# freudh/lbt

Measured on AMD Instinct MI355X. Metric: train-step samples/sec, ResNet-20 CIFAR-10 8-bit DFP, 1/2/4/8 MI355X, higher is better.
Workload: dtype int8; 1 GPU; ResNet-20 CIFAR-10 8-bit DFXP W/A/G train step (fwd+bwd+SGD-momentum+range update); global_batch=128, per_gpu_batch=128, parallelism=dp1, hip_graph=True, executor=fused, grad_range=-6, loss_diverged=False

## Files before the change

lbt_amd/csrc/conv_fused.h:

```cpp
#pragma once
#include "chain_flags.h"
#include "conv_epilogue.h"
#include "lds_tr.h"
#include "pk2.h"

namespace {
using namespace lbt;

#ifdef LBT_P1STUDY
#define LBT_TSS(i) LBT_TS(i)
#define LBT_TSB(i) do { if ((i) == 1) LBT_TS(4); else if ((i) == 2) LBT_TS(5); } while (0)
#else
#define LBT_TSS(i) do { } while (0)
#define LBT_TSB(i) LBT_TS(i)
#endif
constexpr int kBNW = 8;
constexpr int kBThreads = kBNW * 64;
__host__ __device__ constexpr int tile_rows(int CS) { return CS == 1 ? 8 : 4; }
__host__ __device__ constexpr int halo_iters(int TH) { return ((TH + 2) * 128 + kBThreads - 1) / kBThreads; }
template <int CS_, int TH_>
struct FusedTile {
  static constexpr int CS = CS_, TH = TH_, C = CS * 16, C4 = C / 4, W = 512 / C, Wp = W + 2, NT = CS;
  static constexpr int kMaxKS = (9 * CS + 3) / 4;
  static constexpr int NQ = TH * 128, J = (NQ + kBThreads - 1) / kBThreads, NPR = 2 * TH;
  static constexpr int kBIt = halo_iters(TH);
  static_assert(TH % 4 == 0 || TH == 2, "whole groups of 4 rows, or 2-row tiles");
};

template <int C, int KS, bool W4>
struct WImg {
  static constexpr int kBpf = W4 ? 8 : 16;
  static constexpr int kColB = KS * kBpf;
  static constexpr int kStride = kColB + 16;
  static constexpr int kBytes = C * kStride;
  static constexpr int kChunks = C * kColB / 16;
  static constexpr int kIt = (kChunks + kBThreads - 1) / kBThreads;
  static_assert(kColB % 16 == 0, "16-byte chunks within a column");
  LBT_DEV static void load(const int8_t* src, v4i (&v)[kIt]) {
#pragma unroll
    for (int it = 0; it < kIt; ++it) {
      const int i = (int)threadIdx.x + it * kBThreads;
      v[it] = *reinterpret_cast<const v4i*>(src + (int64_t)(i < kChunks ? i : 0) * 16);
    }
  }
  LBT_DEV static void store(int8_t* lds, const v4i (&v)[kIt]) {
#pragma unroll
    for (int it = 0; it < kIt; ++it) {
      const int i = (int)threadIdx.x + it * kBThreads;
      if (i < kChunks) {
        const int g = i * 16, col = g / kColB;
        *reinterpret_cast<v4i*>(lds + col * kStride + (g - col * kColB)) = v[it];
      }
    }
  }
  LBT_DEV static v4i frag(const int8_t* lds, int col, int slice) {
    if constexpr (W4)
      return unpack_i4x16(*reinterpret_cast<const v2i*>(lds + col * kStride + slice * 8));
    else
      return *reinterpret_cast<const v4i*>(lds + col * kStride + slice * 16);
  }
};

template <int C, int TH>
LBT_DEV void halo_pad_fill(int8_t* img, int row0, int H, int word) {
  constexpr int C4 = C / 4, W = 512 / C, Wp = W + 2;
  constexpr int kSide = (TH + 2) * 2 * C4;
  static_assert(kSide <= kBThreads && W * C4 <= kBThreads, "one padding word per thread and kind");
  const int t = kBThreads - 1 - (int)threadIdx.x;
  if (t < kSide) {
    const int hy = t / (2 * C4), side = (t / C4) & 1, q = t % C4;
    *reinterpret_cast<int*>(img + (hy * Wp + side * (W + 1)) * C + q * 4) = word;
  }
  if (t < W * C4) {
    if (row0 == 0) *reinterpret_cast<int*>(img + C + t * 4) = word;
    if (row0 + TH >= H) *reinterpret_cast<int*>(img + ((TH + 1) * Wp + 1) * C + t * 4) = word;
  }
}

LBT_DEV int mask_count(bool p) { return __builtin_popcountll(__builtin_amdgcn_ballot_w64(p)); }
LBT_DEV float max_raw(float a, float b) {
  float r;
  asm("v_max_f32 %0, %1, %2" : "=v"(r) : "v"(a), "v"(b));
  return r;
}
LBT_DEV void ov_count2(pf2 xm, float T1, float T2, int& c) {
  const pf2 n = xm * pk(-0x1.fffffep-1f, -0x1.fffffep-1f);
  const float a0 = max_raw(xm.x, n.x), a1 = max_raw(xm.y, n.y);
  c += mask_count(a0 >= T1) + mask_count(a1 >= T1) + ((mask_count(a0 >= T2) + mask_count(a1 >= T2)) << 16);
  asm volatile("" : "+s"(c));
}
LBT_DEV void ov_count2_pos(pf2 xm, float T1, float T2, int& c) {
  c += mask_count(xm.x >= T1) + mask_count(xm.y >= T1) + ((mask_count(xm.x >= T2) + mask_count(xm.y >= T2)) << 16);
  asm volatile("" : "+s"(c));
}
LBT_DEV void ov_stage_w(int i, int nq, int c, int* sh) {
  counts_stage_w(i, nq, c & 0xffff, (int)((unsigned)c >> 16), sh);
}
LBT_DEV float ov_thr(bool cnt, float T) { return cnt ? T : __builtin_nanf(""); }
constexpr int kOvNan = 0x7fc00000;
LBT_DEV float ov_thr(int nanmask, float T) { return __int_as_float(__float_as_int(T) | nanmask); }

LBT_DEV pf2 qfloor2(const QState& s, pf2 xm, pf2 u) {
  const pf2 v = xm + u;
  return pk(floorf(clip_q(s, v.x)), floorf(clip_q(s, v.y)));
}
LBT_DEV int pack4f(pf2 a, pf2 b) {
  const int c[4] = {(int)a.x, (int)a.y, (int)b.x, (int)b.y};
  return pack4_i8(c);
}

inline bool noise_ok(const lbt_qdesc& q) { return q.bits > 0 && q.stochastic && q.noise; }

}
```

lbt_amd/csrc/conv_fused_bwd.hip:

```cpp
#include "conv_fused.h"
#include "conv_wgrad_body.h"

using namespace lbt;

LBT_TRACE_SETTER(conv_bwd)

namespace {

struct ConvBwdArgs {
  lbt_chain_bwd_b b;
  const int8_t* wd;
  int ks, nslices, w4;
  lbt_qdesc qw;
  int H, W;
  const float* add_src;
  lbt_chain_bwd_a a;
};

template <int C, int TH, int WB>
struct BwdShared {
  int8_t w[WB];
  int8_t gq[(TH + 2) * (512 / C + 2) * C];
  float tile[TH * (512 / C) * (C + 4)];
  float pb[2 * C];
  int part[kBNW][(2 * 4 + 2) * C];
  int cnt[kBNW * 2 * 5];
};

template <int CS, int CF, int NB, bool W4, int WCS, int TH = tile_rows(CS)>
__global__ __launch_bounds__(kBThreads, (CS == 4 && TH >= 4) ? 2 : 4) void conv_bwd_kernel(ConvBwdArgs p, WgradArgs wa, uint32_t nwg) {
  using T = FusedTile<CS, TH>;
  constexpr int C = T::C, C4 = T::C4, NT = T::NT, W = T::W, Wp = T::Wp, kMaxKS = T::kMaxKS;
  constexpr int kBIt = T::kBIt, NPR = T::NPR, NQ = T::NQ, J = T::J;
  constexpr int WC = WCS ? WCS : 1;
  using WI = WImg<C, 4 * kMaxKS, W4>;
  union Smem {
    BwdShared<C, TH, WI::kBytes> b;
    WgradShared<WC, kBNW> w;
  };
  __shared__ __attribute__((aligned(16))) Smem sm;
  if (WCS != 0 && blockIdx.x < nwg) {
    conv_wgrad_body<WC, kBNW>(wa, blockIdx.x, sm.w);
    return;
  }
  BwdShared<C, TH, WI::kBytes>& sh = sm.b;
  LBT_TS(0);
  const lbt_chain_bwd_b& B = p.b;
  const lbt_chain_bwd_a& A = p.a;
  const int H = p.H;
  const uint32_t bid = blockIdx.x - nwg;
  const int tpi = H / TH;
  const int n = (int)(bid / (uint32_t)tpi), row0 = (int)(bid - (uint32_t)n * tpi) * TH;
  const int tid = threadIdx.x, lane = tid & 63, wave = tid >> 6;
  const int r = lane & 15, kg = lane >> 4;
  const int cq = (tid % C4) * 4;
  const int64_t img = (int64_t)n * H * W * C;

  static_assert(LBT_NSHARD == 32 && kBThreads == 512 && C % 16 == 0 && C / 16 <= kBNW, "statistics layout");
  constexpr int kSW = C / 16;
  long long sv[8][2];
  if (wave < kSW) {
    const int64_t* ps = B.sums + (int64_t)(8 * (lane >> 4)) * 4 * C + wave * 16 + (lane & 15);
#pragma unroll
    for (int i = 0; i < 8; ++i) {
      sv[i][0] = ps[(int64_t)i * 4 * C + 2 * C];
      sv[i][1] = ps[(int64_t)i * 4 * C + 3 * C];
    }
  }
  LBT_TSS(1);
  const int ylo = row0 > 0 ? row0 - 1 : 0, yhi = row0 + TH < H ? row0 + TH : H - 1;
  const int ngrp = (yhi - ylo + 1) * W * C4;
  int Gv[kBIt], Qv[kBIt];
  float4 Uv[kBIt];
#pragma unroll
  for (int it = 0; it < kBIt; ++it) {
    const int g = tid + it * kBThreads;
    const uint32_t off = g < ngrp ? (uint32_t)((ylo * W + g / C4) * C + cq) : 0u;
    Gv[it] = ld_i8x4(B.G, img + off);
    Qv[it] = ld_i8x4(B.qn_codes, img + off);
    Uv[it] = ld_f32x4(B.qo.noise, off);
  }
  v4i wimg[WI::kIt];
  WI::load(p.wd, wimg);
  float mu[4], sg[4], gam[2][4], bet[4];
#pragma unroll
  for (int k = 0; k < 4; ++k) {
    mu[k] = B.ms[cq + k];
    sg[k] = B.ms[C + cq + k];
#pragma unroll
    for (int b = 0; b < NB; ++b) gam[b][k] = (b == 0 ? A.b1 : A.b2).gb[cq + k];
    bet[k] = A.b1.gb[C + cq + k];
  }
  const QState sgq = qstate(B.qng), sn = qstate(B.qn), so = qstate(B.qo);
  QState qrg[2], qng[2];
#pragma unroll
  for (int b = 0; b < NB; ++b) {
    qrg[b] = qstate((b == 0 ? A.b1 : A.b2).qrg);
    qng[b] = qstate((b == 0 ? A.b1 : A.b2).qng);
  }
  const float r_inv = (CF & kAMaskR) ? qstate(A.b1.qr).inv_m : 0.f;
  const float scale = ldexpf(1.0f, -(frac_exp(B.qo) + frac_exp(p.qw)));
  LBT_TSS(2);

  if (wave < kSW) {
    long long SGi = 0, SGQi = 0;
#pragma unroll
    for (int i = 0; i < 8; ++i) {
      SGi += sv[i][0];
      SGQi += sv[i][1];
    }
    SGi = rows_total64(SGi);
    SGQi = rows_total64(SGQi);
    const int c = wave * 16 + (lane & 15);
    if (lane < 16) {
      const double s = (double)sn.inv_m, gsc = (double)sgq.inv_m, nn = (double)B.n;
      const double SG = (double)SGi, SGQ = (double)SGQi;
      const float m = B.ms[c], sig = B.ms[C + c];
      sh.pb[c] = (float)(gsc * SG / nn);
      sh.pb[C + c] = (float)(gsc * (s * SGQ - (double)m * SG) / (nn * (double)sig));
    }
  }
  LBT_TSS(3);
  __syncthreads();
  LBT_TSB(1);
  float rmg[4], rmgx[4];
  Recip rsg[4];
#pragma unroll
  for (int k = 0; k < 4; ++k) {
    rmg[k] = sh.pb[cq + k];
    rmgx[k] = sh.pb[C + cq + k];
    rsg[k] = recip(sg[k]);
  }
  pf2 mu2[2], sg2[2], rsc2[2], rmg2[2], rmgx2[2];
#pragma unroll
  for (int h = 0; h < 2; ++h) {
    mu2[h] = pk(mu[2 * h], mu[2 * h + 1]);
    sg2[h] = pk(rsg[2 * h].y, rsg[2 * h + 1].y);
    rsc2[h] = pk(rsg[2 * h].rc, rsg[2 * h + 1].rc);
    rmg2[h] = pk(rmg[2 * h], rmg[2 * h + 1]);
    rmgx2[h] = pk(rmgx[2 * h], rmgx[2 * h + 1]);
  }

  const int wu = __builtin_amdgcn_readfirstlane(wave);
  int ovq = 0;
  int s1[4] = {0, 0, 0, 0}, s2[4] = {0, 0, 0, 0};
#pragma unroll
  for (int it = 0; it < kBIt; ++it) {
    if (it * kBThreads + wu * 64 >= ngrp) break;
    const int g = tid + it * kBThreads;
    const int ry = g / (W * C4), x = g / C4 - ry * W;
    const int y = ylo + ry, hy = y - row0 + 1;
    const int pix = hy * Wp + x + 1;
    const bool own = hy >= 1 && hy <= TH;
    const int hyw = ylo + (it * kBThreads + wu * 64) / (W * C4) - row0 + 1;
    const int nanw = hyw >= 1 && hyw <= TH ? 0 : kOvNan;
    const float T1 = ov_thr(nanw, so.L), T2 = ov_thr(nanw, so.Lh);
    int G[4], q[4], c[4];
    unpack4_i8(Gv[it], G);
    unpack4_i8(Qv[it], q);
    const pf2 u[2] = {pk(Uv[it].x, Uv[it].y), pk(Uv[it].z, Uv[it].w)};
#pragma unroll
    for (int h = 0; h < 2; ++h) {
      const pf2 x1 = pcvt(q[2 * h], q[2 * h + 1]) * sn.inv_m;
      const pf2 x2 = x1 - mu2[h];
      const pf2 xh = pdiv_nz(x2, sg2[h], rsc2[h]);
      const pf2 gh = pcvt(G[2 * h], G[2 * h + 1]) * sgq.inv_m;
      const pf2 t1 = gh - rmg2[h];
      const pf2 t2 = xh * rmgx2[h];
      const pf2 dx = pdiv_nz(t1 - t2, sg2[h], rsc2[h]);
      const pf2 xm = dx * so.m;
      ov_count2(xm, T1, T2, ovq);
      const pf2 fl = qfloor2(so, xm, u[h]);
      c[2 * h] = (int)fl.x;
      c[2 * h + 1] = (int)fl.y;
    }
    *reinterpret_cast<int*>(sh.gq + pix * C + cq) = pack4_i8(c);
    if (own) {
      st_out(B.gq + img + (uint32_t)((y * W + x) * C + cq), pack4_i8(c));
#pragma unroll
      for (int k = 0; k < 4; ++k) {
        s1[k] += c[k];
        s2[k] += c[k] * c[k];
      }
    }
  }
  halo_pad_fill<C, TH>(sh.gq, row0, H, 0);
  WI::store(sh.w, wimg);
  __syncthreads();
  LBT_TSB(2);

  float4 av[J], ymv[J], urg[NB][J], ung[NB][J];
  int Rv[NB][J], qnv[NB][J];
#pragma unroll
  for (int j = 0; j < J; ++j) {
    const int q3 = tid + j * kBThreads;
    const int pix = (q3 < NQ ? q3 : 0) / C4;
    const uint32_t off = (uint32_t)(row0 * W * C + pix * C + cq);
    av[j] = p.add_src ? ld_f32x4(p.add_src, img + off) : make_float4(0.f, 0.f, 0.f, 0.f);
    if (CF & kAYMask) ymv[j] = ld_f32x4(A.y_mask, img + off);
#pragma unroll
    for (int b = 0; b < NB; ++b) {
      const lbt_bwd_branch& Bb = b == 0 ? A.b1 : A.b2;
      Rv[b][j] = ld_i8x4(Bb.R, img + off);
      qnv[b][j] = ld_i8x4(Bb.qn_codes, img + off);
      urg[b][j] = ld_f32x4(Bb.qrg.noise, off);
      ung[b][j] = ld_f32x4(Bb.qng.noise, off);
    }
  }

#pragma unroll
  for (int pi = 0; pi < (NPR + 7) / 8; ++pi) {
    const int pr = wave + 8 * pi;
    if (NPR % 8 && pr >= NPR) break;
    const int mt = pr / NT, nt = pr - mt * NT;
    const int m = mt * 16 + r;
    const int ly = m / W, px = m - ly * W;
    const int8_t* base = sh.gq + ((ly + 2) * Wp + px + 2) * C;
    v4i acc = v4i{0, 0, 0, 0};
    const int col = nt * 16 + r;
#pragma unroll
    for (int kk = 0; kk < kMaxKS; ++kk) {
      const int s = kk * 4 + kg;
      const int tap = s / CS, cs = s - tap * CS;
      const int kh = tap / 3, kw = tap - kh * 3;
      v4i a = *reinterpret_cast<const v4i*>(base - (kh * Wp + kw) * C + cs * 16);
      if (s >= 9 * CS) a = v4i{0, 0, 0, 0};
      acc = __builtin_amdgcn_mfma_i32_16x16x64_i8(a, WI::frag(sh.w, col, s), acc, 0, 0, 0);
    }
#pragma unroll
    for (int i = 0; i < 4; ++i) sh.tile[(mt * 16 + 4 * kg + i) * (C + 4) + nt * 16 + r] = (float)acc[i] * scale;
  }
  __syncthreads();
  LBT_TSB(3);

  int ov[2][2] = {{0, 0}, {0, 0}};
  int acc3[NB][4][4];
#pragma unroll
  for (int b = 0; b < NB; ++b)
#pragma unroll
    for (int s = 0; s < 4; ++s)
#pragma unroll
      for (int k = 0; k < 4; ++k) acc3[b][s][k] = 0;
  const bool has_add = p.add_src != nullptr;
  pf2 gam2a[NB][2], bet2a[2];
#pragma unroll
  for (int h = 0; h < 2; ++h) {
#pragma unroll
    for (int b = 0; b < NB; ++b) gam2a[b][h] = pk(gam[b][2 * h], gam[b][2 * h + 1]);
    bet2a[h] = pk(bet[2 * h], bet[2 * h + 1]);
  }
#pragma unroll
  for (int j = 0; j < J; ++j) {
    if (NQ % kBThreads && wu * 64 + j * kBThreads >= NQ) break;
    const int pix = (tid + j * kBThreads) / C4;
    const uint32_t off = (uint32_t)(row0 * W * C + pix * C + cq);
    const float4 t = *reinterpret_cast<const float4*>(sh.tile + pix * (C + 4) + cq);
    pf2 g[2] = {pk(t.x, t.y), pk(t.z, t.w)};
    if (has_add) {
      g[0] = g[0] + pk(av[j].x, av[j].y);
      g[1] = g[1] + pk(av[j].z, av[j].w);
    }
    int R1[4];
    unpack4_i8(Rv[0][j], R1);
    if (CF & kAYMask) {
      const float ym[4] = {ymv[j].x, ymv[j].y, ymv[j].z, ymv[j].w};
#pragma unroll
      for (int h = 0; h < 2; ++h)
        g[h] = pk(ym[2 * h] > 0.f ? g[h].x : 0.f, ym[2 * h + 1] > 0.f ? g[h].y : 0.f);
    } else if (CF & kAMaskR) {
#pragma unroll
      for (int h = 0; h < 2; ++h) {
        const pf2 xr = pcvt(R1[2 * h], R1[2 * h + 1]) * r_inv;
        const pf2 m1 = xr * gam2a[0][h];
        const pf2 yv = m1 + bet2a[h];
        g[h] = pk(yv.x > 0.f ? g[h].x : 0.f, yv.y > 0.f ? g[h].y : 0.f);
      }
    }
    if (CF & kAGmask) st_out4(A.gmask_out, (uint32_t)(img + off), make_float4(g[0].x, g[0].y, g[1].x, g[1].y));
#pragma unroll
    for (int b = 0; b < NB; ++b) {
      const lbt_bwd_branch& Bb = b == 0 ? A.b1 : A.b2;
      int R[4], qn[4], Gc[4];
      unpack4_i8(Rv[b][j], R);
      unpack4_i8(qnv[b][j], qn);
      const pf2 ur[2] = {pk(urg[b][j].x, urg[b][j].y), pk(urg[b][j].z, urg[b][j].w)};
      const pf2 un[2] = {pk(ung[b][j].x, ung[b][j].y), pk(ung[b][j].z, ung[b][j].w)};
#pragma unroll
      for (int h = 0; h < 2; ++h) {
        const pf2 xm = g[h] * qrg[b].m;
        ov_count2(xm, qrg[b].L, qrg[b].Lh, ov[b][0]);
        const pf2 f1 = qfloor2(qrg[b], xm, ur[h]);
        const pf2 gh = f1 * qrg[b].inv_m;
        const pf2 d = gh * gam2a[b][h];
        const pf2 dm = d * qng[b].m;
        ov_count2(dm, qng[b].L, qng[b].Lh, ov[b][1]);
        const pf2 f2c = qfloor2(qng[b], dm, un[h]);
        const int G2[2] = {(int)f1.x, (int)f1.y};
        Gc[2 * h] = (int)f2c.x;
        Gc[2 * h + 1] = (int)f2c.y;
#pragma unroll
        for (int i = 0; i < 2; ++i) {
          const int k = 2 * h + i;
          acc3[b][0][k] += G2[i] * R[k];
          acc3[b][1][k] += G2[i];
          acc3[b][2][k] += Gc[k];
          acc3[b][3][k] += Gc[k] * qn[k];
        }
      }
      st_out(Bb.gout + img + off, pack4_i8(Gc));
    }
  }

  {
    const bool own = (lane & 15) < C4;
    int* part = sh.part[wave] + cq + (lane >> 4);
#pragma unroll
    for (int b = 0; b < NB; ++b)
#pragma unroll
      for (int s = 0; s < 4; ++s) {
        const int t = chan_scatter4(acc3[b][s], C4);
        if (own) part[(b * 4 + s) * C] = t;
      }
    const int t1 = chan_scatter4(s1, C4), t2 = chan_scatter4(s2, C4);
    if (own) {
      part[8 * C] = t1;
      part[9 * C] = t2;
    }
  }
  ov_stage_w(0, 5, ovq, sh.cnt);
#pragma unroll
  for (int b = 0; b < NB; ++b) {
    ov_stage_w(1 + 2 * b, 5, ov[b][0], sh.cnt);
    ov_stage_w(2 + 2 * b, 5, ov[b][1], sh.cnt);
  }
  __syncthreads();
  LBT_TSB(4);
  counts_publish_nw<kBNW>(0, 5, B.qo, sh.cnt);
#pragma unroll
  for (int b = 0; b < NB; ++b) {
    const lbt_bwd_branch& Bb = b == 0 ? A.b1 : A.b2;
    counts_publish_nw<kBNW>(1 + 2 * b, 5, Bb.qrg, sh.cnt);
    counts_publish_nw<kBNW>(2 + 2 * b, 5, Bb.qng, sh.cnt);
  }
  const int shard = shard_id();
  for (int i = tid; i < (NB * 4 + 2) * C; i += kBThreads) {
    const int slot = i < NB * 4 * C ? i : 8 * C + (i - NB * 4 * C);
    long long v = 0;
#pragma unroll
    for (int w = 0; w < kBNW; ++w) v += sh.part[w][slot];
    if (!v) continue;
    int64_t* dst;
    if (i < NB * 4 * C) {
      const int b = i / (4 * C);
      dst = (b == 0 ? A.b1 : A.b2).sums + (int64_t)shard * 4 * C + (i - b * 4 * C);
    } else {
      if (!B.gcolsum) continue;
      dst = B.gcolsum + (int64_t)shard * 2 * C + (i - NB * 4 * C);
    }
    LBT_GADD((unsigned long long*)dst, (unsigned long long)v);
  }
  LBT_TSB(5);
}

}

extern "C" int lbt_conv_bwd_fused_i8(const lbt_conv_bwd* q, void* stream) {
  if (!q) return LBT_EINVAL;
  const lbt_conv_desc& d = q->d;
  const int C = d.Cin;
  if (!desc_ok(d) || d.KH != 3 || d.KW != 3 || d.SH != 1 || d.SW != 1 || d.PT != 1 || d.PB != 1 || d.PL != 1 ||
      d.PR != 1 || d.Ho != d.H || d.Wo != d.W || d.Cout != C || (C != 16 && C != 32 && C != 64) ||
      d.H % tile_rows(C / 16) || d.W * C != 512 || (int64_t)d.N * d.H * 512 >= ((int64_t)1 << 29))
    return LBT_EINVAL;
  const int CS = C / 16;
  const int64_t inner = (int64_t)d.H * d.W * C;
  const lbt_chain_bwd_b& b = q->b;
  if (!b.G || !b.qn_codes || !b.ms || !b.sums || !b.gq || b.dx || !noise_ok(b.qo) || b.C != C || b.rows != d.N ||
      b.inner != inner)
    return LBT_EINVAL;
  const lbt_chain_bwd_a& a = q->a;
  if (a.C != C || a.rows != d.N || a.inner != inner) return LBT_EINVAL;
  const int f = bwd_a_flags(a);
  if ((f & kAFused) != kAFused) return LBT_EINVAL;
  for (int br = 0; br < (a.has_b2 ? 2 : 1); ++br) {
    const lbt_bwd_branch& Bb = br ? a.b2 : a.b1;
    if (!noise_ok(Bb.qrg) || !noise_ok(Bb.qng) || !Bb.gb) return LBT_EINVAL;
  }
  if (q->ksd != 4 * ((9 * CS + 3) / 4) || !q->wd) return LBT_EINVAL;
  if (q->w4 && q->qw.bits > 4) return LBT_EINVAL;
  if (q->b.qo.bits > 8) return LBT_EINVAL;
  WgradArgs wa{};
  uint32_t wblocks = 0;
  int wcs = 0;
  if (q->w.slab) {
    const int e = wgrad_setup(q->w.xq, q->w.x_u8off, q->w.gq, q->w.d, q->w.slab, q->w.nsplit, q->w.nshard, wa, wblocks);
    if (e) return e;
    wcs = q->w.d.Cin / 16;
  }
  ConvBwdArgs p;
  p.b = b; p.wd = q->wd; p.ks = q->ksd; p.nslices = 9 * CS; p.w4 = q->w4; p.qw = q->qw;
  p.H = d.H; p.W = d.W; p.add_src = q->add_src; p.a = a;
  const int th = lbt_conv_fused_tile_rows(C, d.N, d.H);
  const int64_t tiles = (int64_t)d.N * (d.H / th);
  if (tiles + wblocks > 0x7fffffff) return LBT_EINVAL;
  const dim3 grid((unsigned)(tiles + wblocks));
  hipStream_t st = (hipStream_t)stream;
  const int nb = a.has_b2 ? 2 : 1;
#define LBT_BW_TH(CS_, CF_, NB_, WCS_, TH_)                                                                 \
  if (q->w4)                                                                                                \
    hipLaunchKernelGGL((conv_bwd_kernel<CS_, CF_, NB_, true, WCS_, TH_>), grid, dim3(kBThreads), 0, st, p, wa, wblocks); \
  else                                                                                                      \
    hipLaunchKernelGGL((conv_bwd_kernel<CS_, CF_, NB_, false, WCS_, TH_>), grid, dim3(kBThreads), 0, st, p, wa, wblocks);
#define LBT_BW(CS_, CF_, NB_, WCS_)                                                                  \
  if (CS == CS_ && f == (CF_) && nb == NB_ && wcs == WCS_) {                                       \
    if (CS_ == 1 && th == 4) {                                                                     \
      LBT_BW_TH(CS_, CF_, NB_, WCS_, (CS_ == 1 ? 4 : tile_rows(CS_)))                              \
    } else if (th == 2) {                                                                          \
      LBT_BW_TH(CS_, CF_, NB_, WCS_, 2)                                                            \
    } else {                                                                                       \
      LBT_BW_TH(CS_, CF_, NB_, WCS_, tile_rows(CS_))                                               \
    }                                                                                              \
    return (int)hipGetLastError();                                                                 \
  }
#define LBT_BW_CS(CS_)                                          \
  LBT_BW(CS_, kAFused | kAMaskR, 1, 0)                          \
  LBT_BW(CS_, kAFused | kAMaskR, 1, CS_)                        \
  LBT_BW(CS_, kAFused | kAYMask | kAGmask, 1, 0)                \
  LBT_BW(CS_, kAFused | kAYMask | kAGmask, 1, CS_)              \
  LBT_BW(CS_, kAFused | kAYMask, 2, 0)                          \
  LBT_BW(CS_, kAFused | kAYMask, 2, CS_)
  LBT_BW_CS(1)
  LBT_BW_CS(2)
  LBT_BW_CS(4)
  LBT_BW(1, kAFused | kAYMask, 1, 0)
  LBT_BW(1, kAFused | kAYMask, 1, 1)
  LBT_BW(1, kAFused | kAMaskR, 1, 2)
  LBT_BW(2, kAFused | kAMaskR, 1, 4)
#undef LBT_BW_CS
#undef LBT_BW
#undef LBT_BW_TH
  return LBT_EINVAL;
}

namespace {

struct ConvBwd2Args {
  lbt_chain_bwd_b b1, bs;
  const int8_t* wd1;
  const int8_t* wds;
  lbt_qdesc qw1, qws;
  int H;
  lbt_chain_bwd_a a;
};

template <int C, int TH>
struct Bwd2Shared {
  int8_t g1[(TH / 2 + 1) * 512];
  int8_t gs[(TH / 2) * 512];
  float tile[TH * (512 / C) * (C + 4)];
  float cst[2][5][2 * C];
  int part[kBNW][(2 * 4 + 8) * C];
  int cnt[kBNW * 2 * 6];
};

template <int CS, int CF, int NB, bool W4>
__global__ __launch_bounds__(kBThreads, CS == 1 ? 4 : 2) void conv_bwd2_kernel(ConvBwd2Args p) {
  constexpr int TH = tile_rows(CS);
  using T = FusedTile<CS, TH>;
  constexpr int C = T::C, C4 = T::C4, W = T::W, NT = T::NT, Cq = 2 * C, Cq4 = Cq / 4, CSq = 2 * CS;
  constexpr int Wq = W / 2, J = T::J;
  constexpr int kK1 = (9 * CSq + 3) / 4;
  constexpr int NG1 = (TH / 2 + 1) * Wq * Cq4, NGS = (TH / 2) * Wq * Cq4;
  constexpr int kIt = (NG1 + NGS + kBThreads - 1) / kBThreads;
  static_assert(NG1 % 64 == 0 && CSq <= 4 && LBT_NSHARD == 32 && 2 * Cq / 16 <= kBNW, "layout");
  __shared__ __attribute__((aligned(16))) Bwd2Shared<C, TH> sh;
  LBT_TS(0);
  const lbt_chain_bwd_a& A = p.a;
  const int H = p.H, Hq = H / 2;
  const uint32_t bid = blockIdx.x;
  const int tpi = H / TH;
  const int n = (int)(bid / (uint32_t)tpi), r0 = (int)(bid - (uint32_t)n * tpi) * TH, q0 = r0 / 2;
  const int tid = threadIdx.x, lane = tid & 63, wave = tid >> 6;
  const int r = lane & 15, kg = lane >> 4;
  const int cq = (tid % C4) * 4;
  const int cqq = (tid % Cq4) * 4;
  const int64_t img = (int64_t)n * H * W * C, imgq = (int64_t)n * Hq * Wq * Cq;

  constexpr int kSW = 2 * CSq;
  long long sv[8][2];
  if (wave < kSW) {
    const lbt_chain_bwd_b& Bb = wave < CSq ? p.b1 : p.bs;
    const int c = (wave % CSq) * 16 + (lane & 15);
    const int64_t* ps = Bb.sums + (int64_t)(8 * (lane >> 4)) * 4 * Cq + c;
#pragma unroll
    for (int i = 0; i < 8; ++i) {
      sv[i][0] = ps[(int64_t)i * 4 * Cq + 2 * Cq];
      sv[i][1] = ps[(int64_t)i * 4 * Cq + 3 * Cq];
    }
  }
  int Gv[kIt], Qv[kIt];
  float4 Uv[kIt];
#pragma unroll
  for (int it = 0; it < kIt; ++it) {
    const int g = tid + it * kBThreads;
    const bool r1 = g < NG1;
    const int gg = r1 ? g : g - NG1;
    const int pix = gg / Cq4, hy = pix / Wq, x = pix - hy * Wq;
    const int y = r1 ? q0 - 1 + hy : q0 + hy;
    const bool in = (r1 || gg < NGS) && (unsigned)y < (unsigned)Hq;
    const uint32_t off = in ? (uint32_t)((y * Wq + x) * Cq + cqq) : 0u;
    const lbt_chain_bwd_b& Bb = r1 ? p.b1 : p.bs;
    Gv[it] = ld_i8x4(Bb.G, imgq + off);
    Qv[it] = ld_i8x4(Bb.qn_codes, imgq + off);
    Uv[it] = ld_f32x4(Bb.qo.noise, off);
  }
  v4i bf1[kK1], bfs;
  {
    const int col = (wave % NT) * 16 + r;
#pragma unroll
    for (int kk = 0; kk < kK1; ++kk) {
      if constexpr (W4)
        bf1[kk] = unpack_i4x16(*reinterpret_cast<const v2i*>(p.wd1 + ((int64_t)col * (4 * kK1) + kk * 4 + kg) * 8));
      else
        bf1[kk] = *reinterpret_cast<const v4i*>(p.wd1 + ((int64_t)col * (4 * kK1) + kk * 4 + kg) * 16);
    }
    if constexpr (W4)
      bfs = unpack_i4x16(*reinterpret_cast<const v2i*>(p.wds + ((int64_t)col * 4 + kg) * 8));
    else
      bfs = *reinterpret_cast<const v4i*>(p.wds + ((int64_t)col * 4 + kg) * 16);
  }
  float gam[NB][4], bet[4];
#pragma unroll
  for (int k = 0; k < 4; ++k) {
#pragma unroll
    for (int b = 0; b < NB; ++b) gam[b][k] = (b == 0 ? A.b1 : A.b2).gb[cq + k];
    bet[k] = A.b1.gb[C + cq + k];
  }
  const QState so1 = qstate(p.b1.qo), sos = qstate(p.bs.qo);
  QState qrg[2], qng[2];
#pragma unroll
  for (int b = 0; b < NB; ++b) {
    qrg[b] = qstate((b == 0 ? A.b1 : A.b2).qrg);
    qng[b] = qstate((b == 0 ? A.b1 : A.b2).qng);
  }
  const float r_inv = (CF & kAMaskR) ? qstate(A.b1.qr).inv_m : 0.f;
  const float scale1 = ldexpf(1.0f, -(frac_exp(p.b1.qo) + frac_exp(p.qw1)));
  const float scale2 = ldexpf(1.0f, -(frac_exp(p.bs.qo) + frac_exp(p.qws)));

  if (wave < kSW) {
    long long SGi = 0, SGQi = 0;
#pragma unroll
    for (int i = 0; i < 8; ++i) {
      SGi += sv[i][0];
      SGQi += sv[i][1];
    }
    SGi = rows_total64(SGi);
    SGQi = rows_total64(SGQi);
    const int bn = wave < CSq ? 0 : 1, c = (wave % CSq) * 16 + (lane & 15);
    if (lane < 16) {
      const lbt_chain_bwd_b& Bb = bn == 0 ? p.b1 : p.bs;
      const double s = (double)qstate(Bb.qn).inv_m, gsc = (double)qstate(Bb.qng).inv_m, nn = (double)Bb.n;
      const double SG = (double)SGi, SGQ = (double)SGQi;
      const float m = Bb.ms[c], sig = Bb.ms[Cq + c];
      const Recip rc = recip(sig);
      sh.cst[bn][0][c] = m;
      sh.cst[bn][1][c] = sig;
      sh.cst[bn][2][c] = rc.rc;
      sh.cst[bn][3][c] = (float)(gsc * SG / nn);
      sh.cst[bn][4][c] = (float)(gsc * (s * SGQ - (double)m * SG) / (nn * (double)sig));
    }
  }
  const QState sn1 = qstate(p.b1.qn), sns = qstate(p.bs.qn), sg1 = qstate(p.b1.qng), sgs = qstate(p.bs.qng);
  __syncthreads();
  LBT_TS(1);

  int ova = 0, ovb = 0;
  const int g0w = __builtin_amdgcn_readfirstlane(tid) & ~63;
  int s1a[4] = {0, 0, 0, 0}, s2a[4] = {0, 0, 0, 0}, s1b[4] = {0, 0, 0, 0}, s2b[4] = {0, 0, 0, 0};
#pragma unroll
  for (int it = 0; it < kIt; ++it) {
    if (it * kBThreads >= NG1 + NGS) break;
    const int g = tid + it * kBThreads;
    const bool r1 = g < NG1;
    const int gg = r1 ? g : g - NG1;
    const bool valid = r1 || gg < NGS;
    const int pix = gg / Cq4, hy = pix / Wq, x = pix - hy * Wq;
    const int y = r1 ? q0 - 1 + hy : q0 + hy;
    const bool in = valid && (unsigned)y < (unsigned)Hq;
    const bool own = in && (!r1 || hy >= 1);
    const int bn = r1 ? 0 : 1;
    const QState& so = r1 ? so1 : sos;
    const QState& sn = r1 ? sn1 : sns;
    const QState& sgq = r1 ? sg1 : sgs;
    const float4 mu4 = *reinterpret_cast<const float4*>(&sh.cst[bn][0][cqq]);
    const float4 sg4 = *reinterpret_cast<const float4*>(&sh.cst[bn][1][cqq]);
    const float4 rc4 = *reinterpret_cast<const float4*>(&sh.cst[bn][2][cqq]);
    const float4 mg4 = *reinterpret_cast<const float4*>(&sh.cst[bn][3][cqq]);
    const float4 mx4 = *reinterpret_cast<const float4*>(&sh.cst[bn][4][cqq]);
    const pf2 mu2[2] = {pk(mu4.x, mu4.y), pk(mu4.z, mu4.w)}, sg2[2] = {pk(sg4.x, sg4.y), pk(sg4.z, sg4.w)};
    const pf2 rc2[2] = {pk(rc4.x, rc4.y), pk(rc4.z, rc4.w)}, mg2[2] = {pk(mg4.x, mg4.y), pk(mg4.z, mg4.w)};
    const pf2 mx2[2] = {pk(mx4.x, mx4.y), pk(mx4.z, mx4.w)};
    const float T1 = ov_thr(own, so.L), T2 = ov_thr(own, so.Lh);
    int G[4], q[4], c[4];
    unpack4_i8(Gv[it], G);
    unpack4_i8(Qv[it], q);
    const pf2 u[2] = {pk(Uv[it].x, Uv[it].y), pk(Uv[it].z, Uv[it].w)};
    int o = 0;
#pragma unroll
    for (int h = 0; h < 2; ++h) {
      const pf2 x1 = pcvt(q[2 * h], q[2 * h + 1]) * sn.inv_m;
      const pf2 x2 = x1 - mu2[h];
      const pf2 xh = pdiv_nz(x2, sg2[h], rc2[h]);
      const pf2 gh = pcvt(G[2 * h], G[2 * h + 1]) * sgq.inv_m;
      const pf2 t1 = gh - mg2[h];
      const pf2 t2 = xh * mx2[h];
      const pf2 dx = pdiv_nz(t1 - t2, sg2[h], rc2[h]);
      const pf2 xm = dx * so.m;
      ov_count2(xm, T1, T2, o);
      const pf2 fl = qfloor2(so, xm, u[h]);
      c[2 * h] = in ? (int)fl.x : 0;
      c[2 * h + 1] = in ? (int)fl.y : 0;
    }
    const int w = pack4_i8(c);
    const bool r1w = it * kBThreads + g0w < NG1;
    ova += r1w ? o : 0;
    ovb += r1w ? 0 : o;
    if (r1) {
      *reinterpret_cast<int*>(sh.g1 + pix * Cq + cqq) = w;
      if (own) {
        st_out(p.b1.gq + imgq + (uint32_t)((y * Wq + x) * Cq + cqq), w);
#pragma unroll
        for (int k = 0; k < 4; ++k) {
          s1a[k] += c[k];
          s2a[k] += c[k] * c[k];
        }
      }
    } else {
      if (valid) *reinterpret_cast<int*>(sh.gs + pix * Cq + cqq) = w;
      if (own) {
        st_out(p.bs.gq + imgq + (uint32_t)((y * Wq + x) * Cq + cqq), w);
#pragma unroll
        for (int k = 0; k < 4; ++k) {
          s1b[k] += c[k];
          s2b[k] += c[k] * c[k];
        }
      }
    }
  }
  __syncthreads();
  LBT_TS(2);

  float4 ymv[J], urg[NB][J], ung[NB][J];
  int Rv[NB][J], qnv[NB][J];
#pragma unroll
  for (int j = 0; j < J; ++j) {
    const int pix = (tid + j * kBThreads) / C4;
    const uint32_t off = (uint32_t)(r0 * W * C + pix * C + cq);
    if (CF & kAYMask) ymv[j] = ld_f32x4(A.y_mask, img + off);
#pragma unroll
    for (int b = 0; b < NB; ++b) {
      const lbt_bwd_branch& Bb = b == 0 ? A.b1 : A.b2;
      Rv[b][j] = ld_i8x4(Bb.R, img + off);
      qnv[b][j] = ld_i8x4(Bb.qn_codes, img + off);
      urg[b][j] = ld_f32x4(Bb.qrg.noise, off);
      ung[b][j] = ld_f32x4(Bb.qng.noise, off);
    }
  }

#pragma unroll
  for (int pi = 0; pi < TH / 4; ++pi) {
    const int pr = wave + 8 * pi;
    const int mt = pr / NT, nt = pr - mt * NT;
    const int m = mt * 16 + r;
    const int ly = m / W, px = m - ly * W;
    v4i acc = v4i{0, 0, 0, 0}, acc2 = v4i{0, 0, 0, 0};
#pragma unroll
    for (int kk = 0; kk < kK1; ++kk) {
      const int s = kk * 4 + kg;
      const int tap = s / CSq, cs = s - tap * CSq;
      const int kh = tap / 3, kw = tap - kh * 3;
      const bool ok = s < 9 * CSq && ((ly - kh) & 1) == 0 && ((px - kw) & 1) == 0 && px >= kw;
      const int lr = ((ly - kh) >> 1) + 1, ox = (px - kw) >> 1;
      v4i a = *reinterpret_cast<const v4i*>(sh.g1 + (ok ? (lr * Wq + ox) * Cq + cs * 16 : 0));
      if (!ok) a = v4i{0, 0, 0, 0};
      acc = __builtin_amdgcn_mfma_i32_16x16x64_i8(a, bf1[kk], acc, 0, 0, 0);
    }
    {
      const bool ok = kg < CSq && (ly & 1) == 0 && (px & 1) == 0;
      v4i a = *reinterpret_cast<const v4i*>(sh.gs + (ok ? ((ly >> 1) * Wq + (px >> 1)) * Cq + kg * 16 : 0));
      if (!ok) a = v4i{0, 0, 0, 0};
      acc2 = __builtin_amdgcn_mfma_i32_16x16x64_i8(a, bfs, acc2, 0, 0, 0);
    }
#pragma unroll
    for (int i = 0; i < 4; ++i) {
      const float v = (float)acc[i] * scale1, add = (float)acc2[i] * scale2;
      sh.tile[(mt * 16 + 4 * kg + i) * (C + 4) + nt * 16 + r] = v + add;
    }
  }
  __syncthreads();
  LBT_TS(3);

  int ov[2][2] = {{0, 0}, {0, 0}};
  int acc3[NB][4][4];
#pragma unroll
  for (int b = 0; b < NB; ++b)
#pragma unroll
    for (int s = 0; s < 4; ++s)
#pragma unroll
      for (int k = 0; k < 4; ++k) acc3[b][s][k] = 0;
  pf2 gam2a[NB][2], bet2a[2];
#pragma unroll
  for (int h = 0; h < 2; ++h) {
#pragma unroll
    for (int b = 0; b < NB; ++b) gam2a[b][h] = pk(gam[b][2 * h], gam[b][2 * h + 1]);
    bet2a[h] = pk(bet[2 * h], bet[2 * h + 1]);
  }
#pragma unroll
  for (int j = 0; j < J; ++j) {
    const int pix = (tid + j * kBThreads) / C4;
    const uint32_t off = (uint32_t)(r0 * W * C + pix * C + cq);
    const float4 t = *reinterpret_cast<const float4*>(sh.tile + pix * (C + 4) + cq);
    pf2 g[2] = {pk(t.x, t.y), pk(t.z, t.w)};
    int R1[4];
    unpack4_i8(Rv[0][j], R1);
    if (CF & kAYMask) {
      const float ym[4] = {ymv[j].x, ymv[j].y, ymv[j].z, ymv[j].w};
#pragma unroll
      for (int h = 0; h < 2; ++h)
        g[h] = pk(ym[2 * h] > 0.f ? g[h].x : 0.f, ym[2 * h + 1] > 0.f ? g[h].y : 0.f);
    } else if (CF & kAMaskR) {
#pragma unroll
      for (int h = 0; h < 2; ++h) {
        const pf2 xr = pcvt(R1[2 * h], R1[2 * h + 1]) * r_inv;
        const pf2 m1 = xr * gam2a[0][h];
        const pf2 yv = m1 + bet2a[h];
        g[h] = pk(yv.x > 0.f ? g[h].x : 0.f, yv.y > 0.f ? g[h].y : 0.f);
      }
    }
    if (CF & kAGmask) st_out4(A.gmask_out, (uint32_t)(img + off), make_float4(g[0].x, g[0].y, g[1].x, g[1].y));
#pragma unroll
    for (int b = 0; b < NB; ++b) {
      const lbt_bwd_branch& Bb = b == 0 ? A.b1 : A.b2;
      int R[4], qn[4], Gc[4];
      unpack4_i8(Rv[b][j], R);
      unpack4_i8(qnv[b][j], qn);
      const pf2 ur[2] = {pk(urg[b][j].x, urg[b][j].y), pk(urg[b][j].z, urg[b][j].w)};
      const pf2 un[2] = {pk(ung[b][j].x, ung[b][j].y), pk(ung[b][j].z, ung[b][j].w)};
#pragma unroll
      for (int h = 0; h < 2; ++h) {
        const pf2 xm = g[h] * qrg[b].m;
        ov_count2(xm, qrg[b].L, qrg[b].Lh, ov[b][0]);
        const pf2 f1 = qfloor2(qrg[b], xm, ur[h]);
        const pf2 gh = f1 * qrg[b].inv_m;
        const pf2 d = gh * gam2a[b][h];
        const pf2 dm = d * qng[b].m;
        ov_count2(dm, qng[b].L, qng[b].Lh, ov[b][1]);
        const pf2 f2c = qfloor2(qng[b], dm, un[h]);
        const int G2[2] = {(int)f1.x, (int)f1.y};
        Gc[2 * h] = (int)f2c.x;
        Gc[2 * h + 1] = (int)f2c.y;
#pragma unroll
        for (int i = 0; i < 2; ++i) {
          const int k = 2 * h + i;
          acc3[b][0][k] += G2[i] * R[k];
          acc3[b][1][k] += G2[i];
          acc3[b][2][k] += Gc[k];
          acc3[b][3][k] += Gc[k] * qn[k];
        }
      }
      st_out(Bb.gout + img + off, pack4_i8(Gc));
    }
  }

  {
    const bool own = (lane & 15) < C4;
    int* part = sh.part[wave] + cq + (lane >> 4);
#pragma unroll
    for (int b = 0; b < NB; ++b)
#pragma unroll
      for (int s = 0; s < 4; ++s) {
        const int t = chan_scatter4(acc3[b][s], C4);
        if (own) part[(b * 4 + s) * C] = t;
      }
    const bool ownq = (lane & 15) < Cq4;
    int* pq = sh.part[wave] + NB * 4 * C + cqq + (lane >> 4);
    const int t1 = chan_scatter4(s1a, Cq4), t2 = chan_scatter4(s2a, Cq4);
    const int t3 = chan_scatter4(s1b, Cq4), t4 = chan_scatter4(s2b, Cq4);
    if (ownq) {
      pq[0] = t1;
      pq[Cq] = t2;
      pq[2 * Cq] = t3;
      pq[3 * Cq] = t4;
    }
  }
  constexpr int NQ = 2 + 2 * NB;
  ov_stage_w(0, NQ, ova, sh.cnt);
  ov_stage_w(1, NQ, ovb, sh.cnt);
#pragma unroll
  for (int b = 0; b < NB; ++b) {
    ov_stage_w(2 + 2 * b, NQ, ov[b][0], sh.cnt);
    ov_stage_w(3 + 2 * b, NQ, ov[b][1], sh.cnt);
  }
  __syncthreads();
  LBT_TS(4);
  counts_publish_nw<kBNW>(0, NQ, p.b1.qo, sh.cnt);
  counts_publish_nw<kBNW>(1, NQ, p.bs.qo, sh.cnt);
#pragma unroll
  for (int b = 0; b < NB; ++b) {
    const lbt_bwd_branch& Bb = b == 0 ? A.b1 : A.b2;
    counts_publish_nw<kBNW>(2 + 2 * b, NQ, Bb.qrg, sh.cnt);
    counts_publish_nw<kBNW>(3 + 2 * b, NQ, Bb.qng, sh.cnt);
  }
  const int shard = shard_id();
  for (int i = tid; i < NB * 4 * C + 4 * Cq; i += kBThreads) {
    long long v = 0;
#pragma unroll
    for (int w = 0; w < kBNW; ++w) v += sh.part[w][i];
    if (!v) continue;
    int64_t* dst;
    if (i < NB * 4 * C) {
      const int b = i / (4 * C);
      dst = (b == 0 ? A.b1 : A.b2).sums + (int64_t)shard * 4 * C + (i - b * 4 * C);
    } else {
      const int k = i - NB * 4 * C;
      const lbt_chain_bwd_b& Bb = k < 2 * Cq ? p.b1 : p.bs;
      if (!Bb.gcolsum) continue;
      dst = Bb.gcolsum + (int64_t)shard * 2 * Cq + (k < 2 * Cq ? k : k - 2 * Cq);
    }
    LBT_GADD((unsigned long long*)dst, (unsigned long long)v);
  }
  LBT_TS(5);
}

}

extern "C" int lbt_conv_bwd2_fused_i8(const lbt_conv_bwd2* q, void* stream) {
  if (!q) return LBT_EINVAL;
  const lbt_conv_desc &d1 = q->d1, &ds = q->ds;
  const int C = d1.Cin, Cq = d1.Cout;
  if (!desc_ok(d1) || !desc_ok(ds) || d1.KH != 3 || d1.KW != 3 || d1.SH != 2 || d1.SW != 2 || d1.PT != 0 ||
      d1.PL != 0 || ds.KH != 1 || ds.KW != 1 || ds.SH != 2 || ds.SW != 2 || ds.PT != 0 || ds.PL != 0 ||
      (C != 16 && C != 32) || Cq != 2 * C || d1.W * C != 512 || d1.H % 2 || d1.W % 2 || d1.Ho * 2 != d1.H ||
      d1.Wo * 2 != d1.W || d1.H % tile_rows(C / 16) || ds.N != d1.N || ds.H != d1.H || ds.W != d1.W || ds.Cin != C ||
      ds.Cout != Cq || ds.Ho != d1.Ho || ds.Wo != d1.Wo || (int64_t)d1.N * d1.H * 512 >= ((int64_t)1 << 29))
    return LBT_EINVAL;
  const int CS = C / 16;
  const int64_t inq = (int64_t)d1.Ho * d1.Wo * Cq;
  const lbt_chain_bwd_b* bb[2] = {&q->b1, &q->bs};
  for (int i = 0; i < 2; ++i) {
    const lbt_chain_bwd_b& b = *bb[i];
    if (!b.G || !b.qn_codes || !b.ms || !b.sums || !b.gq || b.dx || !noise_ok(b.qo) || b.C != Cq || b.rows != d1.N ||
        b.inner != inq)
      return LBT_EINVAL;
  }
  const lbt_chain_bwd_a& a = q->a;
  if (a.C != C || a.rows != d1.N || a.inner != (int64_t)d1.H * d1.W * C) return LBT_EINVAL;
  const int f = bwd_a_flags(a);
  if ((f & kAFused) != kAFused) return LBT_EINVAL;
  for (int br = 0; br < (a.has_b2 ? 2 : 1); ++br) {
    const lbt_bwd_branch& Bb = br ? a.b2 : a.b1;
    if (!noise_ok(Bb.qrg) || !noise_ok(Bb.qng) || !Bb.gb) return LBT_EINVAL;
  }
  if (q->ksd1 != 4 * ((9 * 2 * CS + 3) / 4) || q->ksds != 4 || !q->wd1 || !q->wds) return LBT_EINVAL;
  if (q->w4 && (q->qw1.bits > 4 || q->qws.bits > 4)) return LBT_EINVAL;
  if (q->b1.qo.bits > 8 || q->bs.qo.bits > 8) return LBT_EINVAL;
  ConvBwd2Args p;
  p.b1 = q->b1; p.bs = q->bs; p.wd1 = q->wd1; p.wds = q->wds; p.qw1 = q->qw1; p.qws = q->qws; p.H = d1.H; p.a = a;
  const int64_t tiles = (int64_t)d1.N * (d1.H / tile_rows(CS));
  if (tiles > 0x7fffffff || (int64_t)d1.N * d1.H * d1.W * C >= ((int64_t)1 << 31)) return LBT_EINVAL;
  hipStream_t st = (hipStream_t)stream;
  const int nb = a.has_b2 ? 2 : 1;
#define LBT_B2(CS_, CF_, NB_)                                                                              \
  if (CS == CS_ && f == (CF_) && nb == NB_) {                                                              \
    if (q->w4)                                                                                             \
      hipLaunchKernelGGL((conv_bwd2_kernel<CS_, CF_, NB_, true>), dim3((unsigned)tiles), dim3(kBThreads), 0, st, p); \
    else                                                                                                   \
      hipLaunchKernelGGL((conv_bwd2_kernel<CS_, CF_, NB_, false>), dim3((unsigned)tiles), dim3(kBThreads), 0, st, p); \
    return (int)hipGetLastError();                                                                         \
  }
  LBT_B2(1, kAFused | kAYMask | kAGmask, 1)
  LBT_B2(2, kAFused | kAYMask | kAGmask, 1)
  LBT_B2(1, kAFused | kAYMask, 1)
  LBT_B2(2, kAFused | kAYMask, 1)
#undef LBT_B2
  return LBT_EINVAL;
}
```

lbt_amd/csrc/conv_fused_fwd.h:

```cpp
#pragma once
#include "conv_fused.h"

namespace lbt {
int conv_fwd_fused_infer(const lbt_conv_fwd* q, hipStream_t st);
int conv_fwd2_fused_infer(const lbt_conv_fwd2* q, hipStream_t st);
}

namespace {

struct ConvFwdArgs {
  lbt_chain_fwd c;
  const int8_t* wf;
  const int32_t* wcolsum;
  lbt_qdesc qw;
  int H;
  int8_t* yq;
  lbt_qdesc qout;
  int64_t* ychsum;
};

template <int C, int TH, int WB, bool INF = false>
struct FwdShared {
  int8_t w[WB];
  int8_t x[(TH + 2) * (512 / C + 2) * C];
  float tile[TH * (512 / C) * (C + 4)];
  float cst[2][2][C];
  int part[INF ? 1 : kBNW][2 * C];
  int cnt[INF ? 1 : kBNW * 2 * 4];
};

__host__ __device__ constexpr int fwd_waves(int CS, int NB, bool W4, int TH, bool INF) {
  return (CS == 4 && TH >= 4) ? 2 : (CS == 2 && NB == 2 && W4 && TH == 2 && !INF) ? 6 : 4;
}
template <int CS, int NB, int F, bool W4, int TH = tile_rows(CS), bool INF = false>
__global__ __launch_bounds__(kBThreads, fwd_waves(CS, NB, W4, TH, INF)) void conv_fwd_fused_kernel(ConvFwdArgs p) {
  using T = FusedTile<CS, TH>;
  constexpr int C = T::C, C4 = T::C4, NT = T::NT, W = T::W, Wp = T::Wp, kMaxKS = T::kMaxKS;
  constexpr int kBIt = T::kBIt, NQ = T::NQ, J = T::J, NPR = T::NPR;
  using WI = WImg<C, 4 * kMaxKS, W4>;
  __shared__ __attribute__((aligned(16))) FwdShared<C, TH, WI::kBytes, INF> sh;
  LBT_TS(0);
  const lbt_chain_fwd& a = p.c;
  const int H = p.H;
  const uint32_t bid = blockIdx.x;
  const int tpi = H / TH;
  const int n = (int)(bid / (uint32_t)tpi), row0 = (int)(bid - (uint32_t)n * tpi) * TH;
  const int tid = threadIdx.x, lane = tid & 63, wave = tid >> 6;
  const int r = lane & 15, kg = lane >> 4;
  const int cq = (tid % C4) * 4;
  const int64_t img = (int64_t)n * H * W * C;
  constexpr bool RES = (F & kFRes) != 0, YST = (F & kFY) != 0;

  static_assert(LBT_NSHARD == 32 && kBThreads == 512 && (NB * C) % 16 == 0 && NB * C / 16 <= kBNW,
                "moments layout");
  constexpr int kSW = NB * C / 16;
  long long sv[8][2];
  float rmean = 0.f, rvar = 0.f;
  if constexpr (INF) {
    if (tid < NB * C) {
      const lbt_bn_norm& nb = tid < C ? a.b1.nrm : a.b2.nrm;
      rmean = nb.run_mean[tid % C];
      rvar = nb.run_var[tid % C];
    }
  } else if (wave < kSW) {
    const int bc = wave * 16 + (lane & 15), b = bc / C, c = bc - b * C;
    const int64_t* cs = (b == 0 ? a.b1 : a.b2).nrm.chsum + (int64_t)(8 * (lane >> 4)) * 2 * C + c;
#pragma unroll
    for (int i = 0; i < 8; ++i) {
      sv[i][0] = cs[(int64_t)i * 2 * C];
      sv[i][1] = cs[(int64_t)i * 2 * C + C];
    }
  }
  const int ylo = row0 > 0 ? row0 - 1 : 0, yhi = row0 + TH < H ? row0 + TH : H - 1;
  const int ngrp = (yhi - ylo + 1) * W * C4;
  int qv[NB][kBIt];
  float4 rv[kBIt], nrv[NB][kBIt], nov[kBIt];
#pragma unroll
  for (int it = 0; it < kBIt; ++it) {
    const int g = tid + it * kBThreads;
    const uint32_t off = g < ngrp ? (uint32_t)((ylo * W + g / C4) * C + cq) : 0u;
#pragma unroll
    for (int b = 0; b < NB; ++b) {
      const lbt_chain_branch& Bb = b == 0 ? a.b1 : a.b2;
      qv[b][it] = ld_i8x4(Bb.nrm.q, img + off);
      nrv[b][it] = ld_f32x4(Bb.qr.noise, off);
    }
    if constexpr (RES) rv[it] = ld_f32x4(a.res, img + off);
    nov[it] = ld_f32x4(a.qo1.noise, off);
  }
  v4i wimg[WI::kIt];
  WI::load(p.wf, wimg);
  const int bcol = (wave % NT) * 16 + r;
  const int corr = 128 * p.wcolsum[bcol];
  float gam[NB][4], bet[NB][4];
#pragma unroll
  for (int b = 0; b < NB; ++b)
#pragma unroll
    for (int k = 0; k < 4; ++k) {
      gam[b][k] = (b == 0 ? a.b1 : a.b2).gb[cq + k];
      bet[b][k] = (b == 0 ? a.b1 : a.b2).gb[C + cq + k];
    }
  QState qr[2];
  float sn[2];
#pragma unroll
  for (int b = 0; b < NB; ++b) {
    qr[b] = qstate((b == 0 ? a.b1 : a.b2).qr);
    sn[b] = qscale((b == 0 ? a.b1 : a.b2).nrm.qn);
  }
  const QState so1 = qstate(a.qo1), sq = qstate(p.qout);
  const float scale = ldexpf(1.0f, -(frac_exp(a.qo1) + frac_exp(p.qw)));

  if constexpr (INF) {
    if (tid < NB * C) {
      const float eps = (tid < C ? a.b1.nrm : a.b2.nrm).eps;
      sh.cst[tid / C][0][tid % C] = rmean;
      sh.cst[tid / C][1][tid % C] = sqrtf(rvar + eps);
    }
  } else if (wave < kSW) {
    long long S1 = 0, S2 = 0;
#pragma unroll
    for (int i = 0; i < 8; ++i) {
      S1 += sv[i][0];
      S2 += sv[i][1];
    }
    S1 = rows_total64(S1);
    S2 = rows_total64(S2);
    const int bc = wave * 16 + (lane & 15), b = bc / C, c = bc - b * C;
    if (lane < 16) {
    const lbt_bn_norm& nb = b == 0 ? a.b1.nrm : a.b2.nrm;
    const double s = ldexp(1.0, -frac_exp(nb.qn));
    const double mean_d = (double)S1 * s / (double)nb.n;
    const double var_d = (double)S2 * (s * s) / (double)nb.n - mean_d * mean_d;
    const float m = (float)mean_d, vv = (float)var_d;
    const float sigma = sqrtf(vv + nb.eps);
    sh.cst[b][0][c] = m;
    sh.cst[b][1][c] = sigma;
    if (bid == 0) {
      if (nb.ms) { nb.ms[c] = m; nb.ms[C + c] = sigma; }
      if (nb.run_mean) {
        nb.run_mean[c] = nb.momentum * nb.run_mean[c] + nb.one_minus_momentum * m;
        nb.run_var[c] = nb.momentum * nb.run_var[c] + nb.one_minus_momentum * vv;
      }
    }
    }
  }
  __syncthreads();
  LBT_TS(1);
  float pm[NB][4];
  Recip ps[NB][4];
#pragma unroll
  for (int b = 0; b < NB; ++b)
#pragma unroll
    for (int k = 0; k < 4; ++k) {
      pm[b][k] = sh.cst[b][0][cq + k];
      ps[b][k] = recip(sh.cst[b][1][cq + k]);
    }
  pf2 pm2[NB][2], psy2[NB][2], psr2[NB][2], gam2[NB][2], bet2[NB][2];
#pragma unroll
  for (int b = 0; b < NB; ++b)
#pragma unroll
    for (int h = 0; h < 2; ++h) {
      pm2[b][h] = pk(pm[b][2 * h], pm[b][2 * h + 1]);
      psy2[b][h] = pk(ps[b][2 * h].y, ps[b][2 * h + 1].y);
      psr2[b][h] = pk(ps[b][2 * h].rc, ps[b][2 * h + 1].rc);
      gam2[b][h] = pk(gam[b][2 * h], gam[b][2 * h + 1]);
      bet2[b][h] = pk(bet[b][2 * h], bet[b][2 * h + 1]);
    }

  int wu = wave;
  if constexpr (!INF) wu = __builtin_amdgcn_readfirstlane(wave);
  int ovr[2] = {0, 0}, ovx = 0;
#pragma unroll
  for (int it = 0; it < kBIt; ++it) {
    if (it * kBThreads + wu * 64 >= ngrp) break;
    const int g = tid + it * kBThreads;
    const int ry = g / (W * C4), x = g / C4 - ry * W;
    const int y = ylo + ry, hy = y - row0 + 1;
    const int pix = hy * Wp + x + 1;
    const bool own = hy >= 1 && hy <= TH;
    const int hyw = ylo + (it * kBThreads + wu * 64) / (W * C4) - row0 + 1;
    const int nanw = hyw >= 1 && hyw <= TH ? 0 : kOvNan;
    const uint32_t e = (uint32_t)((y * W + x) * C + cq);
    pf2 v[2];
    float T1[2], T2[2];
    if constexpr (!INF) {
#pragma unroll
      for (int b = 0; b < NB; ++b) {
        T1[b] = ov_thr(nanw, qr[b].L);
        T2[b] = ov_thr(nanw, qr[b].Lh);
      }
    }
#pragma unroll
    for (int b = 0; b < NB; ++b) {
      const lbt_chain_branch& Bb = b == 0 ? a.b1 : a.b2;
      int q[4];
      unpack4_i8(qv[b][it], q);
      const pf2 u[2] = {pk(nrv[b][it].x, nrv[b][it].y), pk(nrv[b][it].z, nrv[b][it].w)};
      pf2 fl[2];
#pragma unroll
      for (int h = 0; h < 2; ++h) {
        const pf2 x1 = pcvt(q[2 * h], q[2 * h + 1]) * sn[b];
        const pf2 x2 = x1 - pm2[b][h];
        const pf2 t = pdiv_nz(x2, psy2[b][h], psr2[b][h]);
        const pf2 xm = t * qr[b].m;
        if constexpr (!INF) ov_count2(xm, T1[b], T2[b], ovr[b]);
        fl[h] = qfloor2(qr[b], xm, u[h]);
        const pf2 xr = fl[h] * qr[b].inv_m;
        const pf2 m1 = xr * gam2[b][h];
        const pf2 tt = m1 + bet2[b][h];
        v[h] = b ? v[h] + tt : tt;
      }
      if (own && (!INF || Bb.rout)) st_out(Bb.rout + img + e, pack4f(fl[0], fl[1]));
    }
    if constexpr (RES) {
      v[0] = v[0] + pk(rv[it].x, rv[it].y);
      v[1] = v[1] + pk(rv[it].z, rv[it].w);
    }
#pragma unroll
    for (int h = 0; h < 2; ++h) v[h] = pk(v[h].x > 0.f ? v[h].x : 0.f, v[h].y > 0.f ? v[h].y : 0.f);
    if (YST && own) st_out4(a.y, (uint32_t)(img + e), make_float4(v[0].x, v[0].y, v[1].x, v[1].y));
    const pf2 uo[2] = {pk(nov[it].x, nov[it].y), pk(nov[it].z, nov[it].w)};
    const float X1 = ov_thr(nanw, so1.L), X2 = ov_thr(nanw, so1.Lh);
    int co[4];
#pragma unroll
    for (int h = 0; h < 2; ++h) {
      const pf2 xm = v[h] * so1.m;
      if constexpr (!INF) ov_count2_pos(xm, X1, X2, ovx);
      const pf2 w = xm + uo[h];
      co[2 * h] = floor_i(fminf(w.x, so1.Lm1));
      co[2 * h + 1] = floor_i(fminf(w.y, so1.Lm1));
    }
    const int cw = pack4_i8(co) ^ (int)0x80808080;
    *reinterpret_cast<int*>(sh.x + pix * C + cq) = cw;
    if (own && (!INF || a.o1)) st_out((int8_t*)a.o1 + img + e, cw);
  }
  halo_pad_fill<C, TH>(sh.x, row0, H, (int)0x80808080);
  WI::store(sh.w, wimg);
  __syncthreads();
  LBT_TS(2);
  float4 u3[J];
#pragma unroll
  for (int j = 0; j < J; ++j) {
    const int q3 = tid + j * kBThreads;
    u3[j] = ld_f32x4(p.qout.noise, (uint32_t)(row0 * W * C + ((q3 < NQ ? q3 : 0) / C4) * C + cq));
  }

#pragma unroll
  for (int pi = 0; pi < (NPR + 7) / 8; ++pi) {
    const int pr = wave + 8 * pi;
    if (NPR % 8 && pr >= NPR) break;
    const int mt = pr / NT, nt = pr - mt * NT;
    const int m = mt * 16 + r;
    const int ly = m / W, px = m - ly * W;
    const int8_t* base = sh.x + (ly * Wp + px) * C;
    v4i acc = v4i{0, 0, 0, 0};
#pragma unroll
    for (int kk = 0; kk < kMaxKS; ++kk) {
      const int s = kk * 4 + kg;
      const int tap = s / CS, cs = s - tap * CS;
      const int kh = tap / 3, kw = tap - kh * 3;
      v4i av = *reinterpret_cast<const v4i*>(base + (kh * Wp + kw) * C + cs * 16);
      if (s >= 9 * CS) av = v4i{0, 0, 0, 0};
      acc = __builtin_amdgcn_mfma_i32_16x16x64_i8(av, WI::frag(sh.w, nt * 16 + r, s), acc, 0, 0, 0);
    }
#pragma unroll
    for (int i = 0; i < 4; ++i)
      sh.tile[(mt * 16 + 4 * kg + i) * (C + 4) + nt * 16 + r] = (float)(acc[i] + corr) * scale;
  }
  __syncthreads();
  LBT_TS(3);

  int ovq = 0;
  int s1[4] = {0, 0, 0, 0}, s2[4] = {0, 0, 0, 0};
#pragma unroll
  for (int j = 0; j < J; ++j) {
    if (NQ % kBThreads && (INF ? tid : wu * 64) + j * kBThreads >= NQ) break;
    const int pix3 = (tid + j * kBThreads) / C4;
    const float4 t = *reinterpret_cast<const float4*>(sh.tile + pix3 * (C + 4) + cq);
    const pf2 tv[2] = {pk(t.x, t.y), pk(t.z, t.w)};
    const pf2 u[2] = {pk(u3[j].x, u3[j].y), pk(u3[j].z, u3[j].w)};
    pf2 fl[2];
#pragma unroll
    for (int h = 0; h < 2; ++h) {
      const pf2 xm = tv[h] * sq.m;
      if constexpr (!INF) ov_count2(xm, sq.L, sq.Lh, ovq);
      fl[h] = qfloor2(sq, xm, u[h]);
    }
    const int c[4] = {(int)fl[0].x, (int)fl[0].y, (int)fl[1].x, (int)fl[1].y};
    if constexpr (!INF) {
#pragma unroll
      for (int k = 0; k < 4; ++k) {
        s1[k] += c[k];
        s2[k] += c[k] * c[k];
      }
    }
    st_out(p.yq + img + (uint32_t)(row0 * W * C + pix3 * C + cq), pack4_i8(c));
  }
  if constexpr (!INF) {
    {
      const int t1 = chan_scatter4(s1, C4), t2 = chan_scatter4(s2, C4);
      if ((lane & 15) < C4) {
        sh.part[wave][cq + (lane >> 4)] = t1;
        sh.part[wave][C + cq + (lane >> 4)] = t2;
      }
    }
#pragma unroll
    for (int b = 0; b < NB; ++b) ov_stage_w(b, 4, ovr[b], sh.cnt);
    ov_stage_w(2, 4, ovx, sh.cnt);
    ov_stage_w(3, 4, ovq, sh.cnt);
    __syncthreads();
    LBT_TS(4);
#pragma unroll
    for (int b = 0; b < NB; ++b) counts_publish_nw<kBNW>(b, 4, (b == 0 ? a.b1 : a.b2).qr, sh.cnt);
    counts_publish_nw<kBNW>(2, 4, a.qo1, sh.cnt);
    counts_publish_nw<kBNW>(3, 4, p.qout, sh.cnt);
    if (p.ychsum && tid < 2 * C) {
      long long t = 0;
#pragma unroll
      for (int w = 0; w < kBNW; ++w) t += sh.part[w][tid];
      if (t) LBT_GADD((unsigned long long*)&p.ychsum[(int64_t)shard_id() * 2 * C + tid], (unsigned long long)t);
    }
  }
  LBT_TS(5);
}

constexpr int kTH2 = 4;

struct ConvFwd2Args {
  lbt_chain_fwd c;
  const int8_t* wf1;
  const int8_t* wfs;
  const int32_t* wcolsum1;
  const int32_t* wcolsums;
  lbt_qdesc qw1, qws;
  int H;
  int8_t* yq1;
  int8_t* yqs;
  lbt_qdesc qout1, qouts;
  int64_t* ychsum1;
  int64_t* ychsums;
};

template <int C, bool INF = false>
struct Fwd2Shared {
  int8_t xa[(2 * kTH2 + 1) * 512];
  int8_t xs[kTH2 * 256];
  float tile[2][kTH2 * (256 / C) * (2 * C + 4)];
  float cst[2][C];
  int part[INF ? 1 : kBNW][2 * 2 * 2 * C];
  int cnt[INF ? 1 : kBNW * 2 * 5];
};

template <int CS, bool W4, bool INF = false>
__global__ __launch_bounds__(kBThreads, CS == 1 ? 4 : 2) void conv_fwd2_kernel(ConvFwd2Args p) {
  using T = FusedTile<CS, 2 * kTH2>;
  constexpr int C = T::C, C4 = T::C4, W = T::W, Cq = 2 * C, Cq4 = Cq / 4, Wq = W / 2, NTq = Cq / 16;
  constexpr int kK1 = T::kMaxKS;
  constexpr int NG = (2 * kTH2 + 1) * W * C4;
  constexpr int kIt = (NG + kBThreads - 1) / kBThreads;
  static_assert(kTH2 * Wq * Cq == 2 * 1024 && C / 16 <= kBNW, "layout");
  __shared__ __attribute__((aligned(16))) Fwd2Shared<C, INF> sh;
  LBT_TS(0);
  const lbt_chain_fwd& a = p.c;
  const int H = p.H, Hq = H / 2;
  const uint32_t bid = blockIdx.x;
  const int tpi = Hq / kTH2;
  const int n = (int)(bid / (uint32_t)tpi), oy0 = (int)(bid - (uint32_t)n * tpi) * kTH2, y0 = 2 * oy0;
  const int tid = threadIdx.x, lane = tid & 63, wave = tid >> 6;
  const int r = lane & 15, kg = lane >> 4;
  const int cq = (tid % C4) * 4, cqq = (tid % Cq4) * 4;
  const int64_t img = (int64_t)n * H * W * C, imgq = (int64_t)n * Hq * Wq * Cq;

  constexpr int kSW = C / 16;
  long long sv[8][2];
  float rmean = 0.f, rvar = 0.f;
  if constexpr (INF) {
    if (tid < C) {
      rmean = a.b1.nrm.run_mean[tid];
      rvar = a.b1.nrm.run_var[tid];
    }
  } else if (wave < kSW) {
    const int c = wave * 16 + (lane & 15);
    const int64_t* cs = a.b1.nrm.chsum + (int64_t)(8 * (lane >> 4)) * 2 * C + c;
#pragma unroll
    for (int i = 0; i < 8; ++i) {
      sv[i][0] = cs[(int64_t)i * 2 * C];
      sv[i][1] = cs[(int64_t)i * 2 * C + C];
    }
  }
  int qv[kIt];
  float4 rv[kIt], nrv[kIt], no1[kIt], no2[kIt];
#pragma unroll
  for (int it = 0; it < kIt; ++it) {
    const int g = tid + it * kBThreads;
    const int pix = g / C4, hy = pix / W, x = pix - hy * W;
    const int y = y0 + hy;
    const bool in = g < NG && y < H;
    const uint32_t off = in ? (uint32_t)((y * W + x) * C + cq) : 0u;
    qv[it] = ld_i8x4(a.b1.nrm.q, img + off);
    nrv[it] = ld_f32x4(a.b1.qr.noise, off);
    rv[it] = ld_f32x4(a.res, img + off);
    no1[it] = ld_f32x4(a.qo1.noise, off);
    no2[it] = ld_f32x4(a.qo2.noise, off);
  }
  const int mt = wave / NTq, nt = wave - mt * NTq;
  const int bcol = nt * 16 + r;
  v4i bf1[kK1], bfs;
#pragma unroll
  for (int kk = 0; kk < kK1; ++kk) {
    if constexpr (W4)
      bf1[kk] = unpack_i4x16(*reinterpret_cast<const v2i*>(p.wf1 + ((int64_t)bcol * (4 * kK1) + kk * 4 + kg) * 8));
    else
      bf1[kk] = *reinterpret_cast<const v4i*>(p.wf1 + ((int64_t)bcol * (4 * kK1) + kk * 4 + kg) * 16);
  }
  if constexpr (W4)
    bfs = unpack_i4x16(*reinterpret_cast<const v2i*>(p.wfs + ((int64_t)bcol * 4 + kg) * 8));
  else
    bfs = *reinterpret_cast<const v4i*>(p.wfs + ((int64_t)bcol * 4 + kg) * 16);
  const int corr1 = 128 * p.wcolsum1[bcol], corr2 = 128 * p.wcolsums[bcol];
  float gam[4], bet[4];
#pragma unroll
  for (int k = 0; k < 4; ++k) {
    gam[k] = a.b1.gb[cq + k];
    bet[k] = a.b1.gb[C + cq + k];
  }
  const QState qr = qstate(a.b1.qr), so1 = qstate(a.qo1), so2 = qstate(a.qo2);
  const QState sq1 = qstate(p.qout1), sqs = qstate(p.qouts);
  const float sn = qscale(a.b1.nrm.qn);
  const float scale1 = ldexpf(1.0f, -(frac_exp(a.qo1) + frac_exp(p.qw1)));
  const float scale2 = ldexpf(1.0f, -(frac_exp(a.qo2) + frac_exp(p.qws)));

  if constexpr (INF) {
    if (tid < C) {
      sh.cst[0][tid] = rmean;
      sh.cst[1][tid] = sqrtf(rvar + a.b1.nrm.eps);
    }
  } else if (wave < kSW) {
    long long S1 = 0, S2 = 0;
#pragma unroll
    for (int i = 0; i < 8; ++i) {
      S1 += sv[i][0];
      S2 += sv[i][1];
    }
    S1 = rows_total64(S1);
    S2 = rows_total64(S2);
    const int c = wave * 16 + (lane & 15);
    if (lane < 16) {
      const lbt_bn_norm& nb = a.b1.nrm;
      const double s = ldexp(1.0, -frac_exp(nb.qn));
      const double mean_d = (double)S1 * s / (double)nb.n;
      const double var_d = (double)S2 * (s * s) / (double)nb.n - mean_d * mean_d;
      const float m = (float)mean_d, vv = (float)var_d;
      const float sigma = sqrtf(vv + nb.eps);
      sh.cst[0][c] = m;
      sh.cst[1][c] = sigma;
      if (bid == 0) {
        if (nb.ms) { nb.ms[c] = m; nb.ms[C + c] = sigma; }
        if (nb.run_mean) {
          nb.run_mean[c] = nb.momentum * nb.run_mean[c] + nb.one_minus_momentum * m;
          nb.run_var[c] = nb.momentum * nb.run_var[c] + nb.one_minus_momentum * vv;
        }
      }
    }
  }
  __syncthreads();
  LBT_TS(1);
  pf2 pm2[2], psy2[2], psr2[2], gam2[2], bet2[2];
#pragma unroll
  for (int h = 0; h < 2; ++h) {
    const Recip r0 = recip(sh.cst[1][cq + 2 * h]), r1 = recip(sh.cst[1][cq + 2 * h + 1]);
    pm2[h] = pk(sh.cst[0][cq + 2 * h], sh.cst[0][cq + 2 * h + 1]);
    psy2[h] = pk(r0.y, r1.y);
    psr2[h] = pk(r0.rc, r1.rc);
    gam2[h] = pk(gam[2 * h], gam[2 * h + 1]);
    bet2[h] = pk(bet[2 * h], bet[2 * h + 1]);
  }

  int ovr = 0, ovx = 0, ovs = 0;
#pragma unroll
  for (int it = 0; it < kIt; ++it) {
    if (it * kBThreads >= NG) break;
    const int g = tid + it * kBThreads;
    const int pix = g / C4, hy = pix / W, x = pix - hy * W;
    const int y = y0 + hy;
    const bool valid = g < NG;
    const bool in = valid && y < H;
    const bool own = in && hy < 2 * kTH2;
    const uint32_t e = (uint32_t)((y * W + x) * C + cq);
    int q[4];
    unpack4_i8(qv[it], q);
    const pf2 u[2] = {pk(nrv[it].x, nrv[it].y), pk(nrv[it].z, nrv[it].w)};
    const float T1 = ov_thr(own, qr.L), T2 = ov_thr(own, qr.Lh);
    pf2 fl[2], v[2];
#pragma unroll
    for (int h = 0; h < 2; ++h) {
      const pf2 x1 = pcvt(q[2 * h], q[2 * h + 1]) * sn;
      const pf2 x2 = x1 - pm2[h];
      const pf2 t = pdiv_nz(x2, psy2[h], psr2[h]);
      const pf2 xm = t * qr.m;
      if constexpr (!INF) ov_count2(xm, T1, T2, ovr);
      fl[h] = qfloor2(qr, xm, u[h]);
      const pf2 xr = fl[h] * qr.inv_m;
      const pf2 m1 = xr * gam2[h];
      v[h] = m1 + bet2[h];
    }
    if (own && (!INF || a.b1.rout)) st_out(a.b1.rout + img + e, pack4f(fl[0], fl[1]));
    v[0] = v[0] + pk(rv[it].x, rv[it].y);
    v[1] = v[1] + pk(rv[it].z, rv[it].w);
#pragma unroll
    for (int h = 0; h < 2; ++h) v[h] = pk(v[h].x > 0.f ? v[h].x : 0.f, v[h].y > 0.f ? v[h].y : 0.f);
    if (own) st_out4(a.y, (uint32_t)(img + e), make_float4(v[0].x, v[0].y, v[1].x, v[1].y));
    const pf2 u1[2] = {pk(no1[it].x, no1[it].y), pk(no1[it].z, no1[it].w)};
    const pf2 u2[2] = {pk(no2[it].x, no2[it].y), pk(no2[it].z, no2[it].w)};
    const float X1 = ov_thr(own, so1.L), X2 = ov_thr(own, so1.Lh);
    const float Z1 = ov_thr(own, so2.L), Z2 = ov_thr(own, so2.Lh);
    int c1[4], c2[4];
#pragma unroll
    for (int h = 0; h < 2; ++h) {
      const pf2 xm = v[h] * so1.m;
      if constexpr (!INF) ov_count2_pos(xm, X1, X2, ovx);
      const pf2 w1 = xm + u1[h];
      c1[2 * h] = floor_i(fminf(w1.x, so1.Lm1));
      c1[2 * h + 1] = floor_i(fminf(w1.y, so1.Lm1));
      const pf2 zm = v[h] * so2.m;
      if constexpr (!INF) ov_count2_pos(zm, Z1, Z2, ovs);
      const pf2 w2 = zm + u2[h];
      c2[2 * h] = floor_i(fminf(w2.x, so2.Lm1));
      c2[2 * h + 1] = floor_i(fminf(w2.y, so2.Lm1));
    }
    const int cw1 = in ? (pack4_i8(c1) ^ (int)0x80808080) : (int)0x80808080;
    const int cw2 = in ? (pack4_i8(c2) ^ (int)0x80808080) : (int)0x80808080;
    if (valid) *reinterpret_cast<int*>(sh.xa + pix * C + cq) = cw1;
    if (own && !(hy & 1) && !(x & 1)) *reinterpret_cast<int*>(sh.xs + ((hy >> 1) * Wq + (x >> 1)) * C + cq) = cw2;
    if constexpr (INF) {
      if (own && a.o1) st_out((int8_t*)a.o1 + img + e, cw1);
      if (own && a.o2) st_out((int8_t*)a.o2 + img + e, cw2);
    } else if (own) {
      st_out((int8_t*)a.o1 + img + e, cw1);
      st_out((int8_t*)a.o2 + img + e, cw2);
    }
  }
  __syncthreads();
  LBT_TS(2);
  const uint32_t off3 = (uint32_t)(oy0 * Wq * Cq + (tid / Cq4) * Cq + cqq);
  const float4 un1 = ld_f32x4(p.qout1.noise, off3), uns = ld_f32x4(p.qouts.noise, off3);

  {
    const int m = mt * 16 + r;
    const int ly = m / Wq, px = m - ly * Wq;
    v4i acc = v4i{0, 0, 0, 0}, acc2 = v4i{0, 0, 0, 0};
#pragma unroll
    for (int kk = 0; kk < kK1; ++kk) {
      const int s = kk * 4 + kg;
      const int tap = s / CS, cs = s - tap * CS;
      const int kh = tap / 3, kw = tap - kh * 3;
      const int ix = 2 * px + kw;
      const bool okx = ix < W;
      v4i av = *reinterpret_cast<const v4i*>(sh.xa + (((2 * ly + kh) * W + (okx ? ix : 0)) * C + cs * 16));
      if (!okx) av = v4i{(int)0x80808080, (int)0x80808080, (int)0x80808080, (int)0x80808080};
      if (s >= 9 * CS) av = v4i{0, 0, 0, 0};
      acc = __builtin_amdgcn_mfma_i32_16x16x64_i8(av, bf1[kk], acc, 0, 0, 0);
    }
    {
      v4i av = *reinterpret_cast<const v4i*>(sh.xs + ((ly * Wq + px) * C + (kg < CS ? kg : 0) * 16));
      if (kg >= CS) av = v4i{0, 0, 0, 0};
      acc2 = __builtin_amdgcn_mfma_i32_16x16x64_i8(av, bfs, acc2, 0, 0, 0);
    }
#pragma unroll
    for (int i = 0; i < 4; ++i) {
      const int row = (mt * 16 + 4 * kg + i) * (Cq + 4) + nt * 16 + r;
      sh.tile[0][row] = (float)(acc[i] + corr1) * scale1;
      sh.tile[1][row] = (float)(acc2[i] + corr2) * scale2;
    }
  }
  __syncthreads();
  LBT_TS(3);

  int ovq[2] = {0, 0};
  int s1[2][4] = {{0, 0, 0, 0}, {0, 0, 0, 0}}, s2[2][4] = {{0, 0, 0, 0}, {0, 0, 0, 0}};
  {
    const int pix3 = tid / Cq4;
#pragma unroll
    for (int b = 0; b < 2; ++b) {
      const QState& sq = b ? sqs : sq1;
      const float4 un = b ? uns : un1;
      const float4 t = *reinterpret_cast<const float4*>(sh.tile[b] + pix3 * (Cq + 4) + cqq);
      const pf2 tv[2] = {pk(t.x, t.y), pk(t.z, t.w)};
      const pf2 u[2] = {pk(un.x, un.y), pk(un.z, un.w)};
      pf2 fl[2];
#pragma unroll
      for (int h = 0; h < 2; ++h) {
        const pf2 xm = tv[h] * sq.m;
        if constexpr (!INF) ov_count2(xm, sq.L, sq.Lh, ovq[b]);
        fl[h] = qfloor2(sq, xm, u[h]);
      }
      const int c[4] = {(int)fl[0].x, (int)fl[0].y, (int)fl[1].x, (int)fl[1].y};
      if constexpr (!INF) {
#pragma unroll
        for (int k = 0; k < 4; ++k) {
          s1[b][k] += c[k];
          s2[b][k] += c[k] * c[k];
        }
      }
      st_out((b ? p.yqs : p.yq1) + imgq + off3, pack4_i8(c));
    }
  }
  if constexpr (!INF) {
    {
      const bool ownq = (lane & 15) < Cq4;
#pragma unroll
      for (int b = 0; b < 2; ++b) {
        const int t1 = chan_scatter4(s1[b], Cq4), t2 = chan_scatter4(s2[b], Cq4);
        if (ownq) {
          sh.part[wave][b * 2 * Cq + cqq + (lane >> 4)] = t1;
          sh.part[wave][b * 2 * Cq + Cq + cqq + (lane >> 4)] = t2;
        }
      }
    }
    ov_stage_w(0, 5, ovr, sh.cnt);
    ov_stage_w(1, 5, ovx, sh.cnt);
    ov_stage_w(2, 5, ovs, sh.cnt);
    ov_stage_w(3, 5, ovq[0], sh.cnt);
    ov_stage_w(4, 5, ovq[1], sh.cnt);
    __syncthreads();
    LBT_TS(4);
    counts_publish_nw<kBNW>(0, 5, a.b1.qr, sh.cnt);
    counts_publish_nw<kBNW>(1, 5, a.qo1, sh.cnt);
    counts_publish_nw<kBNW>(2, 5, a.qo2, sh.cnt);
    counts_publish_nw<kBNW>(3, 5, p.qout1, sh.cnt);
    counts_publish_nw<kBNW>(4, 5, p.qouts, sh.cnt);
    if (tid < 4 * Cq) {
      long long t = 0;
#pragma unroll
      for (int w = 0; w < kBNW; ++w) t += sh.part[w][tid];
      int64_t* dst = tid < 2 * Cq ? p.ychsum1 : p.ychsums;
      if (t && dst) LBT_GADD((unsigned long long*)&dst[(int64_t)shard_id() * 2 * Cq + (tid % (2 * Cq))], (unsigned long long)t);
    }
  }
  LBT_TS(5);
}

}
```

lbt_amd/csrc/conv_fused_fwd.hip:

```cpp
#include "conv_fused_fwd.h"
#include "env.h"

using namespace lbt;

LBT_TRACE_SETTER(conv_fwd)

extern "C" int lbt_conv_fused_tile_rows(int32_t Cin, int64_t N, int32_t H) {
  if (Cin != 16 && Cin != 32 && Cin != 64) return -LBT_EINVAL;
  const int CS = Cin / 16;
  if (CS != 1) {
    static const int force23 = getenv_int("LBT_TILE_ROWS23", 0);
    if (force23 == 4 || H % 4) return 4;
    return (force23 == 2 || N * H / 4 < 256) ? 2 : 4;
  }
  static const int force = getenv_int("LBT_TILE_ROWS1", 0);
  if (force == 2 || force == 4 || force == 8) return H % force ? 8 : force;
  if (N * H / 8 >= 256 || H % 4) return 8;
  return (N * H / 4 < 256 && H % 2 == 0) ? 2 : 4;
}

static int frozen_chain(const lbt_chain_fwd& a) {
  const bool f1 = a.b1.nrm.frozen != 0, f2 = a.has_b2 ? a.b2.nrm.frozen != 0 : f1;
  return f1 != f2 ? -1 : (f1 ? 1 : 0);
}

extern "C" int lbt_conv_fwd_fused_i8(const lbt_conv_fwd* q, void* stream) {
  if (!q) return LBT_EINVAL;
  if (const int fz = frozen_chain(q->c)) return fz < 0 ? LBT_EINVAL : conv_fwd_fused_infer(q, (hipStream_t)stream);
  const lbt_conv_desc& d = q->d;
  const int C = d.Cin;
  if (!desc_ok(d) || d.KH != 3 || d.KW != 3 || d.SH != 1 || d.SW != 1 || d.PT != 1 || d.PB != 1 || d.PL != 1 ||
      d.PR != 1 || d.Ho != d.H || d.Wo != d.W || d.Cout != C || (C != 16 && C != 32 && C != 64) ||
      d.H % tile_rows(C / 16) || d.W * C != 512 || (int64_t)d.N * d.H * 512 >= ((int64_t)1 << 29))
    return LBT_EINVAL;
  const int CS = C / 16;
  const lbt_chain_fwd& a = q->c;
  const int64_t inner = (int64_t)d.H * d.W * C;
  if (a.C != C || a.rows != d.N || a.inner != inner || a.o2 || !a.o1 || a.o1_kind != LBT_OUT_U8OFF) return LBT_EINVAL;
  const int f = fwd_flags(a);
  constexpr int kNeed = kFQ | kFRout | kFRelu | kFO1 | kFStoch | kFU8;
  if ((f & kRt) || (f & kNeed) != kNeed || (f & (kFO2 | kFNoR))) return LBT_EINVAL;
  if (!noise_ok(a.qo1)) return LBT_EINVAL;
  for (int br = 0; br < (a.has_b2 ? 2 : 1); ++br) {
    const lbt_chain_branch& Bb = br ? a.b2 : a.b1;
    if (!noise_ok(Bb.qr) || !Bb.gb || !Bb.nrm.chsum || Bb.nrm.frozen) return LBT_EINVAL;
  }
  if (!q->yq || !noise_ok(q->qout) || !q->wcolsum || !q->wf) return LBT_EINVAL;
  if (q->ksf != 4 * ((9 * CS + 3) / 4)) return LBT_EINVAL;
  if (q->w4 && q->qw.bits > 4) return LBT_EINVAL;
  if (q->qout.bits > 8) return LBT_EINVAL;
  ConvFwdArgs p;
  p.c = a; p.wf = q->wf; p.wcolsum = q->wcolsum; p.qw = q->qw; p.H = d.H;
  p.yq = q->yq; p.qout = q->qout; p.ychsum = q->ychsum;
  const int th = lbt_conv_fused_tile_rows(C, d.N, d.H);
  const int64_t tiles = (int64_t)d.N * (d.H / th);
  if (tiles > 0x7fffffff) return LBT_EINVAL;
  const dim3 grid((unsigned)tiles);
  hipStream_t st = (hipStream_t)stream;
  const int nb = a.has_b2 ? 2 : 1;
  const int fl = f & ~kFU8 & ~kFStoch;
#define LBT_FW_TH(CS_, NB_, FL_, TH_)                                                                        \
  if (q->w4)                                                                                                 \
    hipLaunchKernelGGL((conv_fwd_fused_kernel<CS_, NB_, FL_, true, TH_>), grid, dim3(kBThreads), 0, st, p);    \
  else                                                                                                       \
    hipLaunchKernelGGL((conv_fwd_fused_kernel<CS_, NB_, FL_, false, TH_>), grid, dim3(kBThreads), 0, st, p);
#define LBT_FW(CS_, NB_, FL_)                                                                            \
  if (CS == CS_ && nb == NB_ && fl == ((FL_) & ~kFU8 & ~kFStoch)) {                                      \
    if (CS_ == 1 && th == 4) {                                                                           \
      LBT_FW_TH(CS_, NB_, FL_, (CS_ == 1 ? 4 : tile_rows(CS_)))                                          \
    } else if (th == 2) {                                                                                \
      LBT_FW_TH(CS_, NB_, FL_, 2)                                                                        \
    } else {                                                                                             \
      LBT_FW_TH(CS_, NB_, FL_, tile_rows(CS_))                                                           \
    }                                                                                                    \
    return (int)hipGetLastError();                                                                       \
  }
#define LBT_FW_CS(CS_)                                  \
  LBT_FW(CS_, 1, kNeed)                                 \
  LBT_FW(CS_, 1, kNeed | kFRes | kFY)                   \
  LBT_FW(CS_, 2, kNeed | kFY)
  LBT_FW(1, 1, kNeed)
  LBT_FW(1, 1, kNeed | kFRes | kFY)
  LBT_FW(1, 1, kNeed | kFY)
  LBT_FW_CS(2)
  LBT_FW_CS(4)
#undef LBT_FW_CS
#undef LBT_FW
#undef LBT_FW_TH
  return LBT_EINVAL;
}

extern "C" int lbt_conv_fwd2_fused_i8(const lbt_conv_fwd2* q, void* stream) {
  if (!q) return LBT_EINVAL;
  if (const int fz = frozen_chain(q->c)) return fz < 0 ? LBT_EINVAL : conv_fwd2_fused_infer(q, (hipStream_t)stream);
  const lbt_conv_desc &d1 = q->d1, &ds = q->ds;
  const int C = d1.Cin, Cq = d1.Cout;
  if (!desc_ok(d1) || !desc_ok(ds) || d1.KH != 3 || d1.KW != 3 || d1.SH != 2 || d1.SW != 2 || d1.PT != 0 ||
      d1.PL != 0 || ds.KH != 1 || ds.KW != 1 || ds.SH != 2 || ds.SW != 2 || ds.PT != 0 || ds.PL != 0 ||
      (C != 16 && C != 32) || Cq != 2 * C || d1.W * C != 512 || d1.H % 2 || d1.W % 2 || d1.Ho * 2 != d1.H ||
      d1.Wo * 2 != d1.W || d1.Ho % kTH2 || ds.N != d1.N || ds.H != d1.H || ds.W != d1.W || ds.Cin != C ||
      ds.Cout != Cq || ds.Ho != d1.Ho || ds.Wo != d1.Wo || (int64_t)d1.N * d1.H * 512 >= ((int64_t)1 << 29))
    return LBT_EINVAL;
  const int CS = C / 16;
  const lbt_chain_fwd& a = q->c;
  if (a.C != C || a.rows != d1.N || a.inner != (int64_t)d1.H * d1.W * C || a.has_b2 || !a.o1 || !a.o2 ||
      a.o1_kind != LBT_OUT_U8OFF || a.o2_kind != LBT_OUT_U8OFF || !a.res || !a.y)
    return LBT_EINVAL;
  const int f = fwd_flags(a);
  constexpr int kNeed = kFQ | kFRout | kFRelu | kFO1 | kFO2 | kFStoch | kFU8 | kFRes | kFY;
  if (f != kNeed) return LBT_EINVAL;
  if (!noise_ok(a.qo1) || !noise_ok(a.qo2) || !noise_ok(a.b1.qr) || !a.b1.gb || !a.b1.nrm.chsum || a.b1.nrm.frozen)
    return LBT_EINVAL;
  if (!q->yq1 || !q->yqs || !noise_ok(q->qout1) || !noise_ok(q->qouts) || !q->wcolsum1 || !q->wcolsums || !q->wf1 ||
      !q->wfs)
    return LBT_EINVAL;
  if (q->ksf1 != 4 * ((9 * CS + 3) / 4) || q->ksfs != 4) return LBT_EINVAL;
  if (q->w4 && (q->qw1.bits > 4 || q->qws.bits > 4)) return LBT_EINVAL;
  if (q->qout1.bits > 8 || q->qouts.bits > 8) return LBT_EINVAL;
  ConvFwd2Args p;
  p.c = a; p.wf1 = q->wf1; p.wfs = q->wfs; p.wcolsum1 = q->wcolsum1; p.wcolsums = q->wcolsums;
  p.qw1 = q->qw1; p.qws = q->qws; p.H = d1.H; p.yq1 = q->yq1; p.yqs = q->yqs; p.qout1 = q->qout1;
  p.qouts = q->qouts; p.ychsum1 = q->ychsum1; p.ychsums = q->ychsums;
  const int64_t tiles = (int64_t)d1.N * (d1.Ho / kTH2);
  if (tiles > 0x7fffffff || (int64_t)d1.N * d1.H * d1.W * C >= ((int64_t)1 << 31)) return LBT_EINVAL;
  hipStream_t st = (hipStream_t)stream;
#define LBT_F2(CS_)                                                                                           \
  if (CS == CS_) {                                                                                            \
    if (q->w4)                                                                                                \
      hipLaunchKernelGGL((conv_fwd2_kernel<CS_, true>), dim3((unsigned)tiles), dim3(kBThreads), 0, st, p);    \
    else                                                                                                      \
      hipLaunchKernelGGL((conv_fwd2_kernel<CS_, false>), dim3((unsigned)tiles), dim3(kBThreads), 0, st, p);   \
    return (int)hipGetLastError();                                                                            \
  }
  LBT_F2(1)
  LBT_F2(2)
#undef LBT_F2
  return LBT_EINVAL;
}
```

lbt_amd/csrc/conv_fused_infer.hip:

```cpp
#include "conv_fused_fwd.h"

using namespace lbt;

LBT_TRACE_SETTER(conv_infer)

namespace {

bool branch_ok(const lbt_chain_branch& b) {
  return b.nrm.frozen && b.nrm.q && b.nrm.run_mean && b.nrm.run_var && b.gb && noise_ok(b.qr) && !b.qr.counts;
}
bool qout_ok(const lbt_qdesc& q) { return noise_ok(q) && !q.counts; }

}

int lbt::conv_fwd_fused_infer(const lbt_conv_fwd* q, hipStream_t st) {
  const lbt_conv_desc& d = q->d;
  const int C = d.Cin;
  if (!desc_ok(d) || d.KH != 3 || d.KW != 3 || d.SH != 1 || d.SW != 1 || d.PT != 1 || d.PB != 1 || d.PL != 1 ||
      d.PR != 1 || d.Ho != d.H || d.Wo != d.W || d.Cout != C || (C != 16 && C != 32 && C != 64) ||
      d.H % tile_rows(C / 16) || d.W * C != 512 || (int64_t)d.N * d.H * 512 >= ((int64_t)1 << 29))
    return LBT_EINVAL;
  const int CS = C / 16;
  const lbt_chain_fwd& a = q->c;
  if (a.C != C || a.rows != d.N || a.inner != (int64_t)d.H * d.W * C || a.o2 || !a.relu) return LBT_EINVAL;
  if (a.o1 && a.o1_kind != LBT_OUT_U8OFF) return LBT_EINVAL;
  if (!branch_ok(a.b1) || (a.has_b2 && !branch_ok(a.b2)) || !qout_ok(a.qo1)) return LBT_EINVAL;
  if (!q->yq || !qout_ok(q->qout) || q->ychsum || !q->wcolsum || !q->wf) return LBT_EINVAL;
  if (q->ksf != 4 * ((9 * CS + 3) / 4)) return LBT_EINVAL;
  if (q->w4 && q->qw.bits > 4) return LBT_EINVAL;
  ConvFwdArgs p;
  p.c = a; p.wf = q->wf; p.wcolsum = q->wcolsum; p.qw = q->qw; p.H = d.H;
  p.yq = q->yq; p.qout = q->qout; p.ychsum = nullptr;
  const int th = lbt_conv_fused_tile_rows(C, d.N, d.H);
  const int64_t tiles = (int64_t)d.N * (d.H / th);
  if (tiles > 0x7fffffff) return LBT_EINVAL;
  const dim3 grid((unsigned)tiles);
  const int nb = a.has_b2 ? 2 : 1;
  const int fl = (a.res ? kFRes : 0) | (a.y ? kFY : 0);
#define LBT_FI_TH(CS_, NB_, FL_, TH_)                                                                              \
  if (q->w4)                                                                                                       \
    hipLaunchKernelGGL((conv_fwd_fused_kernel<CS_, NB_, FL_, true, TH_, true>), grid, dim3(kBThreads), 0, st, p);  \
  else                                                                                                             \
    hipLaunchKernelGGL((conv_fwd_fused_kernel<CS_, NB_, FL_, false, TH_, true>), grid, dim3(kBThreads), 0, st, p);
#define LBT_FI(CS_, NB_, FL_)                                  \
  if (CS == CS_ && nb == NB_ && fl == (FL_)) {                 \
    if (CS_ == 1 && th == 4) {                                 \
      LBT_FI_TH(CS_, NB_, FL_, (CS_ == 1 ? 4 : tile_rows(CS_))) \
    } else if (th == 2) {                                      \
      LBT_FI_TH(CS_, NB_, FL_, 2)                              \
    } else {                                                   \
      LBT_FI_TH(CS_, NB_, FL_, tile_rows(CS_))                 \
    }                                                          \
    return (int)hipGetLastError();                             \
  }
#define LBT_FI_CS(CS_)            \
  LBT_FI(CS_, 1, 0)               \
  LBT_FI(CS_, 1, kFRes | kFY)     \
  LBT_FI(CS_, 1, kFY)             \
  LBT_FI(CS_, 2, kFY)
  LBT_FI_CS(1)
  LBT_FI_CS(2)
  LBT_FI_CS(4)
#undef LBT_FI_CS
#undef LBT_FI
#undef LBT_FI_TH
  return LBT_EINVAL;
}

int lbt::conv_fwd2_fused_infer(const lbt_conv_fwd2* q, hipStream_t st) {
  const lbt_conv_desc &d1 = q->d1, &ds = q->ds;
  const int C = d1.Cin, Cq = d1.Cout;
  if (!desc_ok(d1) || !desc_ok(ds) || d1.KH != 3 || d1.KW != 3 || d1.SH != 2 || d1.SW != 2 || d1.PT != 0 ||
      d1.PL != 0 || ds.KH != 1 || ds.KW != 1 || ds.SH != 2 || ds.SW != 2 || ds.PT != 0 || ds.PL != 0 ||
      (C != 16 && C != 32) || Cq != 2 * C || d1.W * C != 512 || d1.H % 2 || d1.W % 2 || d1.Ho * 2 != d1.H ||
      d1.Wo * 2 != d1.W || d1.Ho % kTH2 || ds.N != d1.N || ds.H != d1.H || ds.W != d1.W || ds.Cin != C ||
      ds.Cout != Cq || ds.Ho != d1.Ho || ds.Wo != d1.Wo || (int64_t)d1.N * d1.H * 512 >= ((int64_t)1 << 29))
    return LBT_EINVAL;
  const int CS = C / 16;
  const lbt_chain_fwd& a = q->c;
  if (a.C != C || a.rows != d1.N || a.inner != (int64_t)d1.H * d1.W * C || a.has_b2 || !a.res || !a.y || !a.relu)
    return LBT_EINVAL;
  if ((a.o1 && a.o1_kind != LBT_OUT_U8OFF) || (a.o2 && a.o2_kind != LBT_OUT_U8OFF)) return LBT_EINVAL;
  if (!branch_ok(a.b1) || !qout_ok(a.qo1) || !qout_ok(a.qo2)) return LBT_EINVAL;
  if (!q->yq1 || !q->yqs || !qout_ok(q->qout1) || !qout_ok(q->qouts) || q->ychsum1 || q->ychsums || !q->wcolsum1 ||
      !q->wcolsums || !q->wf1 || !q->wfs)
    return LBT_EINVAL;
  if (q->ksf1 != 4 * ((9 * CS + 3) / 4) || q->ksfs != 4) return LBT_EINVAL;
  if (q->w4 && (q->qw1.bits > 4 || q->qws.bits > 4)) return LBT_EINVAL;
  ConvFwd2Args p;
  p.c = a; p.wf1 = q->wf1; p.wfs = q->wfs; p.wcolsum1 = q->wcolsum1; p.wcolsums = q->wcolsums;
  p.qw1 = q->qw1; p.qws = q->qws; p.H = d1.H; p.yq1 = q->yq1; p.yqs = q->yqs; p.qout1 = q->qout1;
  p.qouts = q->qouts; p.ychsum1 = nullptr; p.ychsums = nullptr;
  const int64_t tiles = (int64_t)d1.N * (d1.Ho / kTH2);
  if (tiles > 0x7fffffff || (int64_t)d1.N * d1.H * d1.W * C >= ((int64_t)1 << 31)) return LBT_EINVAL;
#define LBT_F2I(CS_)                                                                                               \
  if (CS == CS_) {                                                                                                 \
    if (q->w4)                                                                                                     \
      hipLaunchKernelGGL((conv_fwd2_kernel<CS_, true, true>), dim3((unsigned)tiles), dim3(kBThreads), 0, st, p);   \
    else                                                                                                           \
      hipLaunchKernelGGL((conv_fwd2_kernel<CS_, false, true>), dim3((unsigned)tiles), dim3(kBThreads), 0, st, p);  \
    return (int)hipGetLastError();                                                                                 \
  }
  LBT_F2I(1)
  LBT_F2I(2)
#undef LBT_F2I
  return LBT_EINVAL;
}
```

lbt_amd/csrc/dfxp_device.h:

```cpp
#pragma once
#include <hip/hip_runtime.h>
#include <stdint.h>

#include <type_traits>

#include "../../include/lbt_dfxp.h"

#define LBT_DEV __device__ __forceinline__

#ifdef LBT_EXP_PLAINSTORE
#define LBT_GADD(p, v) (*(p) = (v))
#else
#define LBT_GADD(p, v) atomicAdd((p), (v))
#endif

#ifdef LBT_TRACE
static __device__ unsigned long long* lbt_trace_buf;
#define LBT_TS(i)                                                                                       \
  do {                                                                                                  \
    if (threadIdx.x == 0 && lbt_trace_buf) {                                                            \
      const size_t wg_ = (size_t)blockIdx.x + (size_t)blockIdx.y * gridDim.x;                           \
      lbt_trace_buf[wg_ * 8 + (i)] = __builtin_amdgcn_s_memrealtime();                                  \
      if ((i) == 0) {                                                                                   \
        unsigned x_;                                                                                    \
        asm volatile("s_getreg_b32 %0, hwreg(HW_REG_XCC_ID)" : "=s"(x_));                               \
        lbt_trace_buf[wg_ * 8 + 7] = x_;                                                                \
      }                                                                                                 \
    }                                                                                                   \
  } while (0)
#define LBT_TROLE(v)                                                                                    \
  do {                                                                                                  \
    if (threadIdx.x == 0 && lbt_trace_buf)                                                              \
      lbt_trace_buf[((size_t)blockIdx.x + (size_t)blockIdx.y * gridDim.x) * 8 + 6] = (v);               \
  } while (0)
#define LBT_TRACE_SETTER(tu)                                                                            \
  extern "C" int lbt_trace_set_##tu(void* p) {                                                          \
    return (int)hipMemcpyToSymbol(HIP_SYMBOL(lbt_trace_buf), &p, sizeof(p));                            \
  }
#else
#define LBT_TS(i) \
  do {            \
  } while (0)
#define LBT_TROLE(v) \
  do {               \
  } while (0)
#define LBT_TRACE_SETTER(tu)
#endif

namespace lbt {

#ifdef LBT_PLAIN_OUT
LBT_DEV void st_out(int* p, int v) { *p = v; }
#else
LBT_DEV void st_out(int* p, int v) { __hip_atomic_store(p, v, __ATOMIC_RELAXED, __HIP_MEMORY_SCOPE_AGENT); }
#endif
#if defined(LBT_PLAIN_OUT) || defined(LBT_PLAIN_OUT4)
LBT_DEV void st_out4(float* base, uint32_t i, float4 v) { *reinterpret_cast<float4*>(base + i) = v; }
#else
LBT_DEV void st_out4(float* base, uint32_t i, float4 v) {
  typedef unsigned int v4u_ __attribute__((ext_vector_type(4)));
  const __amdgpu_buffer_rsrc_t r = __builtin_amdgcn_make_buffer_rsrc(base, 0, 0x7fffffff, 0x00020000);
  const v4u_ x = {__float_as_uint(v.x), __float_as_uint(v.y), __float_as_uint(v.z), __float_as_uint(v.w)};
  __builtin_amdgcn_raw_buffer_store_b128(x, r, (int)(i * 4u), 0, 16 );
}
#endif
LBT_DEV void st_out(int8_t* p, int v) { st_out(reinterpret_cast<int*>(p), v); }
LBT_DEV void st_out(float* p, float v) { st_out(reinterpret_cast<int*>(p), __float_as_int(v)); }
#ifdef LBT_PLAIN_OUT
LBT_DEV void st_out8(void* p, long long v) { *reinterpret_cast<long long*>(p) = v; }
#else
LBT_DEV void st_out8(void* p, long long v) {
  __hip_atomic_store(reinterpret_cast<long long*>(p), v, __ATOMIC_RELAXED, __HIP_MEMORY_SCOPE_AGENT);
}
#endif
#ifdef LBT_WT_TAIL
#define LBT_ST_TAIL(p, v) st_out((p), (v))
#else
#define LBT_ST_TAIL(p, v) (void)(*(p) = (v))
#endif
LBT_DEV void st_out16(float* p, float4 v) {
  st_out8(p, (long long)(((unsigned long long)__float_as_uint(v.y) << 32) | __float_as_uint(v.x)));
  st_out8(p + 2, (long long)(((unsigned long long)__float_as_uint(v.w) << 32) | __float_as_uint(v.z)));
}

constexpr int kEMax = 30;

struct U4 { uint32_t x, y, z, w; };

LBT_DEV U4 philox(uint32_t c0, uint32_t c1, uint32_t c2, uint32_t c3, uint32_t k0, uint32_t k1) {
#pragma unroll
  for (int r = 0; r < 10; ++r) {
    if (r) { k0 += 0x9E3779B9u; k1 += 0xBB67AE85u; }
    const uint32_t lo0 = 0xD2511F53u * c0, hi0 = __umulhi(0xD2511F53u, c0);
    const uint32_t lo1 = 0xCD9E8D57u * c2, hi1 = __umulhi(0xCD9E8D57u, c2);
    const uint32_t n0 = hi1 ^ c1 ^ k0, n2 = hi0 ^ c3 ^ k1;
    c0 = n0; c1 = lo1; c2 = n2; c3 = lo0;
  }
  return U4{c0, c1, c2, c3};
}

LBT_DEV float u24(uint32_t r) { return (float)(r >> 8) * 5.9604644775390625e-8f; }

struct Noise4 { float u[4]; };
LBT_DEV Noise4 noise4(uint64_t blk, uint32_t qid, uint64_t step, uint64_t seed) {
  U4 r = philox((uint32_t)blk, qid, (uint32_t)step, (uint32_t)(step >> 32), (uint32_t)seed,
                (uint32_t)(seed >> 32));
  Noise4 n;
  n.u[0] = u24(r.x); n.u[1] = u24(r.y); n.u[2] = u24(r.z); n.u[3] = u24(r.w);
  return n;
}
LBT_DEV Noise4 qnoise4(const lbt_qdesc& q, uint64_t step, uint64_t blk) {
  if (q.noise) {
    const float4 v = *reinterpret_cast<const float4*>(q.noise + 4 * blk);
    return Noise4{{v.x, v.y, v.z, v.w}};
  }
  return noise4(blk, q.qid, step, q.seed);
}
LBT_DEV float noise1(uint64_t idx, uint32_t qid, uint64_t step, uint64_t seed) {
  U4 r = philox((uint32_t)(idx >> 2), qid, (uint32_t)step, (uint32_t)(step >> 32), (uint32_t)seed,
                (uint32_t)(seed >> 32));
  const uint32_t k = (uint32_t)(idx & 3);
  return u24(k == 0 ? r.x : k == 1 ? r.y : k == 2 ? r.z : r.w);
}
LBT_DEV float qnoise1(const lbt_qdesc& q, uint64_t step, uint64_t idx) {
  return q.noise ? q.noise[idx] : noise1(idx, q.qid, step, q.seed);
}

static __device__ __attribute__((aligned(16))) int32_t kZeroBlock[64];
LBT_DEV const float* zf() { return reinterpret_cast<const float*>(kZeroBlock); }
LBT_DEV const int32_t* zi() { return kZeroBlock; }

struct QState {
  float m, inv_m, L, Lm1, Lh;
  int e;
  uint64_t step;
  int active;
};

LBT_DEV int frac_exp(const lbt_qdesc& q) {
  int e = q.bits - q.exps[q.slot] - 1;
  return e < 0 ? 0 : (e > kEMax ? kEMax : e);
}

LBT_DEV QState qstate(const lbt_qdesc& q) {
  QState s;
  s.active = q.bits > 0;
  const int32_t* ep = s.active ? q.exps + q.slot : zi();
  const uint64_t* sp = (s.active && q.step) ? q.step : reinterpret_cast<const uint64_t*>(zi());
  const int I = *ep;
  const uint64_t st = *sp;
  int e = q.bits - I - 1;
  e = e < 0 ? 0 : (e > kEMax ? kEMax : e);
  s.e = s.active ? e : 0;
  s.m = s.active ? ldexpf(1.0f, e) : 0.f;
  s.inv_m = s.active ? ldexpf(1.0f, -e) : 0.f;
  s.L = s.active ? ldexpf(1.0f, q.bits - 1) : 0.f;
  s.Lm1 = s.active ? s.L - 1.0f : 0.f;
  s.Lh = s.active ? ldexpf(1.0f, q.bits - 2) : 0.f;
  s.step = st;
  return s;
}

LBT_DEV float qscale(const lbt_qdesc& q) { return ldexpf(1.0f, -frac_exp(q)); }

LBT_DEV int wave_id() { return __builtin_amdgcn_readfirstlane((int)(threadIdx.x >> 6)); }

LBT_DEV float ovf_abs(float xm) { return fmaxf(xm, xm * -0x1.fffffep-1f); }
LBT_DEV int floor_i(float v) {
  int r;
  asm("v_cvt_flr_i32_f32 %0, %1" : "=v"(r) : "v"(v));
  return r;
}
LBT_DEV int quant1(const QState& s, int stochastic, float x, float u, int& ov1, int& ov2) {
  const float xm = x * s.m;
  const float a = ovf_abs(xm);
  ov1 += a >= s.L;
  ov2 += a >= s.Lh;
  float v = stochastic ? (xm + u) : xm;
  v = fminf(fmaxf(v, -s.L), s.Lm1);
  v = stochastic ? floorf(v) : rintf(v);
  return (int)v;
}

struct Recip { float y, rc; };
LBT_DEV Recip recip(float y) {
  const float r0 = __builtin_amdgcn_rcpf(y);
  const float e = fmaf(-y, r0, 1.0f);
  return Recip{y, fmaf(e, r0, r0)};
}
LBT_DEV float div_by(float x, const Recip& d) {
  const float q = x * d.rc;
  const float r = fmaf(-d.y, q, x);
  const float q1 = fmaf(r, d.rc, q);
  const float r1 = fmaf(-d.y, q1, x);
  return copysignf(fmaf(r1, d.rc, q1), x);
}


template <int STOCH>
LBT_DEV int quant_w(const QState& s, int stochastic, float x, float u, int& ov1w, int& ov2w) {
  const float xm = x * s.m;
  const float a = ovf_abs(xm);
  ov1w += __popcll(__ballot(a >= s.L));
  ov2w += __popcll(__ballot(a >= s.Lh));
  const bool st = STOCH < 0 ? stochastic != 0 : STOCH == 1;
  float v = st ? (xm + u) : xm;
  v = fminf(fmaxf(v, -s.L), s.Lm1);
  v = st ? floorf(v) : rintf(v);
  return (int)v;
}

LBT_DEV void counts_stage_w(int i, int nq, int ov1w, int ov2w, int* sh) {
  if ((threadIdx.x & 63) == 0) {
    int* p = sh + (threadIdx.x >> 6) * 2 * nq + 2 * i;
    p[0] = ov1w;
    p[1] = ov2w;
  }
}

template <int K>
LBT_DEV int quad_from(int v) {
  if constexpr (K == 0) return v;
  else if constexpr (K == 1) return __builtin_amdgcn_mov_dpp(v, 0x39, 0xf, 0xf, false);
  else if constexpr (K == 2) return __builtin_amdgcn_mov_dpp(v, 0x4E, 0xf, 0xf, false);
  else return __builtin_amdgcn_mov_dpp(v, 0x93, 0xf, 0xf, false);
}
template <int K>
LBT_DEV float quad_from(float v) { return __int_as_float(quad_from<K>(__float_as_int(v))); }
LBT_DEV uint32_t quad_pack_codes(const int (&c)[4], int jj) {
  uint32_t packed = 0;
  auto step = [&](auto kc) {
    constexpr int k = decltype(kc)::value;
    const int sc = (jj - k) & 3;
    const int send = sc == 0 ? c[0] : sc == 1 ? c[1] : sc == 2 ? c[2] : c[3];
    const int got = quad_from<k>(send);
    packed |= ((uint32_t)got & 0xFFu) << (8 * ((jj + k) & 3));
  };
  step(std::integral_constant<int, 0>{});
  step(std::integral_constant<int, 1>{});
  step(std::integral_constant<int, 2>{});
  step(std::integral_constant<int, 3>{});
  return packed;
}

LBT_DEV int wave_sum_i32(int v) {
#pragma unroll
  for (int o = 32; o > 0; o >>= 1) v += __shfl_xor(v, o, 64);
  return v;
}
LBT_DEV long long wave_sum_i64(long long v) {
#pragma unroll
  for (int o = 32; o > 0; o >>= 1) v += __shfl_xor(v, o, 64);
  return v;
}

LBT_DEV int shard_id() {
  return (int)((blockIdx.x + blockIdx.y * 7u + blockIdx.z * 13u) % LBT_NSHARD);
}

LBT_DEV void counts_stage(int i, int nq, int ov1, int ov2, int* sh) {
  ov1 = wave_sum_i32(ov1);
  ov2 = wave_sum_i32(ov2);
  if ((threadIdx.x & 63) == 0) {
    int* p = sh + (threadIdx.x >> 6) * 2 * nq + 2 * i;
    p[0] = ov1;
    p[1] = ov2;
  }
}
LBT_DEV void counts_publish(int i, int nq, const lbt_qdesc& q, const int* sh) {
  const int j = (int)threadIdx.x - 2 * i;
  if (!q.counts || j < 0 || j > 1) return;
  const int nw = (blockDim.x + 63) >> 6;
  int t = 0;
  for (int w = 0; w < nw; ++w) t += sh[w * 2 * nq + 2 * i + j];
  if (t) LBT_GADD(q.counts + ((int64_t)q.slot * LBT_NSHARD + shard_id()) * LBT_CSTRIDE + j, t);
}

template <int NW>
LBT_DEV void counts_publish_nw(int i, int nq, const lbt_qdesc& q, const int* sh) {
  const int j = (int)threadIdx.x - 64 * (i % NW);
  if (!q.counts || j < 0 || j > 1) return;
  int t = 0;
#pragma unroll
  for (int w = 0; w < NW; ++w) t += sh[w * 2 * nq + 2 * i + j];
  if (t) LBT_GADD(q.counts + ((int64_t)q.slot * LBT_NSHARD + shard_id()) * LBT_CSTRIDE + j, t);
}

LBT_DEV void block_flush_counts(const lbt_qdesc& q, int ov1, int ov2, int* sh) {
  if (!q.counts) return;
  counts_stage(0, 1, ov1, ov2, sh);
  __syncthreads();
  counts_publish(0, 1, q, sh);
  __syncthreads();
}

LBT_DEV void block_flush_counts_w(const lbt_qdesc& q, int ov1w, int ov2w, int* sh) {
  if (!q.counts) return;
  counts_stage_w(0, 1, ov1w, ov2w, sh);
  __syncthreads();
  counts_publish(0, 1, q, sh);
  __syncthreads();
}

LBT_DEV void block_flush_sums(const long long* sh, int n, int64_t* dst, int stride) {
  int64_t* d = dst + (int64_t)shard_id() * stride;
  for (int i = threadIdx.x; i < n; i += blockDim.x)
    if (sh[i]) LBT_GADD((unsigned long long*)&d[i], (unsigned long long)sh[i]);
}

LBT_DEV int chan_period(int C) {
  const int p = C >> 2;
  return (C % 4 == 0 && p > 0 && p <= 32 && (p & (p - 1)) == 0) ? p : 0;
}
LBT_DEV int wave_chan_reduce(int v, int period) {
  if (period)
    for (int o = period; o < 64; o <<= 1) v += __shfl_xor(v, o, 64);
  return v;
}
LBT_DEV bool chan_owner(int period) { return period == 0 || (int)(threadIdx.x & 63) < period; }

LBT_DEV int rows_scatter4(int v0, int v1, int v2, int v3) {
  const auto a = __builtin_amdgcn_permlane16_swap(v0, v1, false, false);
  const auto b = __builtin_amdgcn_permlane16_swap(v2, v3, false, false);
  const int p01 = (int)a[0] + (int)a[1], p23 = (int)b[0] + (int)b[1];
  const auto c = __builtin_amdgcn_permlane32_swap(p01, p23, false, false);
  return (int)c[0] + (int)c[1];
}
LBT_DEV int rows_scatter2(int v0, int v1) {
  const auto a = __builtin_amdgcn_permlane16_swap(v0, v1, false, false);
  const int p = (int)a[0] + (int)a[1];
  const auto c = __builtin_amdgcn_permlane32_swap(p, p, false, false);
  return (int)c[0] + (int)c[1];
}
LBT_DEV int chan_scatter4(const int v[4], int period) {
  int t = rows_scatter4(v[0], v[1], v[2], v[3]);
  if (period <= 8) t += __builtin_amdgcn_update_dpp(0, t, 0x128, 0xf, 0xf, false);
  if (period <= 4) t += __builtin_amdgcn_update_dpp(0, t, 0x124, 0xf, 0xf, false);
  if (period <= 2) t += __builtin_amdgcn_update_dpp(0, t, 0x4E, 0xf, 0xf, false);
  if (period <= 1) t += __builtin_amdgcn_update_dpp(0, t, 0xB1, 0xf, 0xf, false);
  return t;
}
LBT_DEV bool chan_scatter_ok(int period) { return period >= 1 && period <= 16; }
LBT_DEV bool chan_scatter_owner(int period) { return (int)(threadIdx.x & 15) < period; }

LBT_DEV int row_pair_sum(int v) {
  const auto h = __builtin_amdgcn_permlane16_swap(v, v, false, false);
  return (int)h[0] + (int)h[1];
}
LBT_DEV int half_pair_sum(int v) {
  const auto h = __builtin_amdgcn_permlane32_swap(v, v, false, false);
  return (int)h[0] + (int)h[1];
}
LBT_DEV long long rows_total64(long long v) {
  const uint32_t lo = (uint32_t)v, hi = (uint32_t)((unsigned long long)v >> 32);
  const auto a = __builtin_amdgcn_permlane16_swap(lo, lo, false, false);
  const auto b = __builtin_amdgcn_permlane16_swap(hi, hi, false, false);
  v = (long long)(((unsigned long long)b[0] << 32) | a[0]) + (long long)(((unsigned long long)b[1] << 32) | a[1]);
  const uint32_t lo2 = (uint32_t)v, hi2 = (uint32_t)((unsigned long long)v >> 32);
  const auto c = __builtin_amdgcn_permlane32_swap(lo2, lo2, false, false);
  const auto d = __builtin_amdgcn_permlane32_swap(hi2, hi2, false, false);
  return (long long)(((unsigned long long)d[0] << 32) | c[0]) + (long long)(((unsigned long long)d[1] << 32) | c[1]);
}

LBT_DEV int ld_i8x4(const int8_t* p, int64_t i) { return *reinterpret_cast<const int*>(p + i); }
LBT_DEV float4 ld_f32x4(const float* p, int64_t i) { return *reinterpret_cast<const float4*>(p + i); }
LBT_DEV void unpack4_i8(int w, int v[4]) {
  v[0] = (int8_t)(w & 0xff); v[1] = (int8_t)((w >> 8) & 0xff);
  v[2] = (int8_t)((w >> 16) & 0xff); v[3] = (int8_t)(w >> 24);
}
LBT_DEV int pack4_i8(const int c[4]) {
  return (int)((uint32_t)(c[0] & 0xff) | ((uint32_t)(c[1] & 0xff) << 8) | ((uint32_t)(c[2] & 0xff) << 16) |
               ((uint32_t)c[3] << 24));
}

LBT_DEV void range_apply(int i, int c1, int c2, int32_t* exps, const int32_t* bits, const float* target,
                         const float* nelem) {
  if (bits[i] >= 32) return;
  const float r1 = (float)c1 / nelem[i];
  const float r2 = (float)c2 / nelem[i];
  const float t = target[i];
  const int delta = r1 > t ? 1 : (r2 <= t ? -1 : 0);
  int I = exps[i] + delta;
  const int hi = bits[i] - 1, lo = bits[i] - 1 - kEMax;
  I = I > hi ? hi : (I < lo ? lo : I);
  exps[i] = I;
}

LBT_DEV bool wave_shard_totals(int32_t* counts, int i, int& c1, int& c2) {
  const int lane = threadIdx.x & 63;
  int a = 0, b = 0;
  if (lane < LBT_NSHARD) {
    int32_t* c = counts + ((int64_t)i * LBT_NSHARD + lane) * LBT_CSTRIDE;
    a = c[0];
    b = c[1];
    c[0] = 0;
    c[1] = 0;
  }
  c1 = wave_sum_i32(a);
  c2 = wave_sum_i32(b);
  return lane == 0;
}

LBT_DEV void sgd_momentum_elem(float* w, float* a, const float* g, int64_t i, float lr, float mu, float gscale) {
  const float t = mu * a[i];
  const float gg = g[i] * gscale;
  const float an = t + gg;
  a[i] = an;
  const float step = lr * an;
  w[i] = w[i] - step;
}

LBT_DEV void store_code(void* out, int kind, int64_t i, int qv, float inv_m) {
  switch (kind) {
    case LBT_OUT_I8: ((int8_t*)out)[i] = (int8_t)qv; break;
    case LBT_OUT_U8OFF: ((int8_t*)out)[i] = (int8_t)((qv < 0 ? 0 : qv) - 128); break;
    case LBT_OUT_I16: ((int16_t*)out)[i] = (int16_t)qv; break;
    default: ((float*)out)[i] = (float)qv * inv_m; break;
  }
}

}
```

Measured before the change: 326,200 samples/s.

## Use buffer loads with scalar row offsets and raise occupancy for small fused conv kernels

Rewrites the address computation in the fused conv forward and backward kernels. Each element offset is split into a wave-uniform scalar row offset plus a per-lane byte offset and issued through raw buffer load/store intrinsics, which cuts per-thread VGPR address arithmetic and 64-bit pointer math. Tile and image indices are made uniform with readfirstlane. It also raises launch_bounds waves-per-EU for specific CS=1 forward and CS=2 backward variants, which could cause register spills. The extent guard is tightened so that 32-bit offsets stay valid.

```diff
diff --git a/lbt_amd/csrc/conv_fused.h b/lbt_amd/csrc/conv_fused.h
--- a/lbt_amd/csrc/conv_fused.h
+++ b/lbt_amd/csrc/conv_fused.h
@@ -26,6 +26,30 @@
   static constexpr int kBIt = halo_iters(TH);
   static_assert(TH % 4 == 0 || TH == 2, "whole groups of 4 rows, or 2-row tiles");
 };
+constexpr uint32_t kRowB = 512;
+LBT_DEV uint32_t lane_off1() { return (threadIdx.x & 127u) * 4u; }
+LBT_DEV int uni(int v) { return __builtin_amdgcn_readfirstlane(v); }
+template <bool UA>
+struct Addr {
+  LBT_DEV static int ld8(const int8_t* p, int64_t img, uint32_t sbyte, uint32_t vbyte) {
+    if constexpr (UA) return ld_i8x4_u(p + img, sbyte, vbyte);
+    else return ld_i8x4(p, img + (sbyte + vbyte));
+  }
+  LBT_DEV static float4 ld32(const float* p, int64_t img, uint32_t sbyte, uint32_t vbyte) {
+    if constexpr (UA) return ld_f32x4_u(p + img, sbyte, vbyte);
+    else return ld_f32x4(p, img + ((sbyte + vbyte) >> 2));
+  }
+  LBT_DEV static void st8(int8_t* p, int64_t img, uint32_t sbyte, uint32_t vbyte, int v) {
+    if constexpr (UA) st_out_u(p + img, sbyte, vbyte, v);
+    else st_out(p + img + (sbyte + vbyte), v);
+  }
+  LBT_DEV static void st32(float* p, int64_t img, uint32_t sbyte, uint32_t vbyte, float4 v) {
+    st_out4(p, ((uint32_t)img + (sbyte >> 2)) + (vbyte >> 2), v);
+  }
+};
+inline bool fused_extent_ok(int64_t N, int64_t H) {
+  return H > 0 && H * 4 * kRowB < ((int64_t)1 << 31) && N * H * kRowB < ((int64_t)1 << 29);
+}
 
 template <int C, int KS, bool W4>
 struct WImg {
diff --git a/lbt_amd/csrc/conv_fused_bwd.hip b/lbt_amd/csrc/conv_fused_bwd.hip
--- a/lbt_amd/csrc/conv_fused_bwd.hip
+++ b/lbt_amd/csrc/conv_fused_bwd.hip
@@ -27,12 +27,16 @@
   int cnt[kBNW * 2 * 5];
 };
 
+__host__ __device__ constexpr int bwd_waves(int CS, int NB, bool W4, int TH) {
+  return (CS == 4 && TH >= 4) ? 2 : (CS == 2 && NB == 2 && W4 && TH == 2) ? 6 : 4;
+}
 template <int CS, int CF, int NB, bool W4, int WCS, int TH = tile_rows(CS)>
-__global__ __launch_bounds__(kBThreads, (CS == 4 && TH >= 4) ? 2 : 4) void conv_bwd_kernel(ConvBwdArgs p, WgradArgs wa, uint32_t nwg) {
+__global__ __launch_bounds__(kBThreads, bwd_waves(CS, NB, W4, TH)) void conv_bwd_kernel(ConvBwdArgs p, WgradArgs wa, uint32_t nwg) {
   using T = FusedTile<CS, TH>;
   constexpr int C = T::C, C4 = T::C4, NT = T::NT, W = T::W, Wp = T::Wp, kMaxKS = T::kMaxKS;
   constexpr int kBIt = T::kBIt, NPR = T::NPR, NQ = T::NQ, J = T::J;
   constexpr int WC = WCS ? WCS : 1;
+  using AD = Addr<NB == 1>;
   using WI = WImg<C, 4 * kMaxKS, W4>;
   union Smem {
     BwdShared<C, TH, WI::kBytes> b;
@@ -50,11 +54,13 @@
   const int H = p.H;
   const uint32_t bid = blockIdx.x - nwg;
   const int tpi = H / TH;
-  const int n = (int)(bid / (uint32_t)tpi), row0 = (int)(bid - (uint32_t)n * tpi) * TH;
+  const int n = uni((int)(bid / (uint32_t)tpi)), row0 = uni((int)(bid - (uint32_t)n * tpi) * TH);
   const int tid = threadIdx.x, lane = tid & 63, wave = tid >> 6;
   const int r = lane & 15, kg = lane >> 4;
   const int cq = (tid % C4) * 4;
-  const int64_t img = (int64_t)n * H * W * C;
+  const int64_t img = (int64_t)n * H * kRowB;
+  const int wu = wave_id();
+  const uint32_t l1 = lane_off1();
 
   static_assert(LBT_NSHARD == 32 && kBThreads == 512 && C % 16 == 0 && C / 16 <= kBNW, "statistics layout");
   constexpr int kSW = C / 16;
@@ -74,11 +80,11 @@
   float4 Uv[kBIt];
 #pragma unroll
   for (int it = 0; it < kBIt; ++it) {
-    const int g = tid + it * kBThreads;
-    const uint32_t off = g < ngrp ? (uint32_t)((ylo * W + g / C4) * C + cq) : 0u;
-    Gv[it] = ld_i8x4(B.G, img + off);
-    Qv[it] = ld_i8x4(B.qn_codes, img + off);
-    Uv[it] = ld_f32x4(B.qo.noise, off);
+    const int gw = it * kBThreads + wu * 64;
+    const uint32_t rowb = gw < ngrp ? (uint32_t)(ylo + gw / 128) * kRowB : 0u;
+    Gv[it] = AD::ld8(B.G, img, rowb, l1);
+    Qv[it] = AD::ld8(B.qn_codes, img, rowb, l1);
+    Uv[it] = AD::ld32(B.qo.noise, 0, rowb * 4u, l1 * 4u);
   }
   v4i wimg[WI::kIt];
   WI::load(p.wd, wimg);
@@ -141,19 +147,15 @@
     rmgx2[h] = pk(rmgx[2 * h], rmgx[2 * h + 1]);
   }
 
-  const int wu = __builtin_amdgcn_readfirstlane(wave);
   int ovq = 0;
   int s1[4] = {0, 0, 0, 0}, s2[4] = {0, 0, 0, 0};
 #pragma unroll
   for (int it = 0; it < kBIt; ++it) {
-    if (it * kBThreads + wu * 64 >= ngrp) break;
-    const int g = tid + it * kBThreads;
-    const int ry = g / (W * C4), x = g / C4 - ry * W;
-    const int y = ylo + ry, hy = y - row0 + 1;
-    const int pix = hy * Wp + x + 1;
+    const int gw = it * kBThreads + wu * 64;
+    if (gw >= ngrp) break;
+    const int y = ylo + gw / 128, hy = y - row0 + 1;
     const bool own = hy >= 1 && hy <= TH;
-    const int hyw = ylo + (it * kBThreads + wu * 64) / (W * C4) - row0 + 1;
-    const int nanw = hyw >= 1 && hyw <= TH ? 0 : kOvNan;
+    const int nanw = own ? 0 : kOvNan;
     const float T1 = ov_thr(nanw, so.L), T2 = ov_thr(nanw, so.Lh);
     int G[4], q[4], c[4];
     unpack4_i8(Gv[it], G);
@@ -174,9 +176,9 @@
       c[2 * h] = (int)fl.x;
       c[2 * h + 1] = (int)fl.y;
     }
-    *reinterpret_cast<int*>(sh.gq + pix * C + cq) = pack4_i8(c);
+    *reinterpret_cast<int*>(sh.gq + (hy * Wp + 1) * C + l1) = pack4_i8(c);
     if (own) {
-      st_out(B.gq + img + (uint32_t)((y * W + x) * C + cq), pack4_i8(c));
+      AD::st8(B.gq, img, (uint32_t)y * kRowB, l1, pack4_i8(c));
 #pragma unroll
       for (int k = 0; k < 4; ++k) {
         s1[k] += c[k];
@@ -191,20 +193,19 @@
 
   float4 av[J], ymv[J], urg[NB][J], ung[NB][J];
   int Rv[NB][J], qnv[NB][J];
+  const uint32_t l3 = (NQ % kBThreads && tid >= NQ) ? (uint32_t)cq : (uint32_t)tid * 4u;
 #pragma unroll
   for (int j = 0; j < J; ++j) {
-    const int q3 = tid + j * kBThreads;
-    const int pix = (q3 < NQ ? q3 : 0) / C4;
-    const uint32_t off = (uint32_t)(row0 * W * C + pix * C + cq);
-    av[j] = p.add_src ? ld_f32x4(p.add_src, img + off) : make_float4(0.f, 0.f, 0.f, 0.f);
-    if (CF & kAYMask) ymv[j] = ld_f32x4(A.y_mask, img + off);
+    const uint32_t t3 = (uint32_t)row0 * kRowB + j * 4 * kBThreads;
+    av[j] = p.add_src ? AD::ld32(p.add_src, img, t3 * 4u, l3 * 4u) : make_float4(0.f, 0.f, 0.f, 0.f);
+    if (CF & kAYMask) ymv[j] = AD::ld32(A.y_mask, img, t3 * 4u, l3 * 4u);
 #pragma unroll
     for (int b = 0; b < NB; ++b) {
       const lbt_bwd_branch& Bb = b == 0 ? A.b1 : A.b2;
-      Rv[b][j] = ld_i8x4(Bb.R, img + off);
-      qnv[b][j] = ld_i8x4(Bb.qn_codes, img + off);
-      urg[b][j] = ld_f32x4(Bb.qrg.noise, off);
-      ung[b][j] = ld_f32x4(Bb.qng.noise, off);
+      Rv[b][j] = AD::ld8(Bb.R, img, t3, l3);
+      qnv[b][j] = AD::ld8(Bb.qn_codes, img, t3, l3);
+      urg[b][j] = AD::ld32(Bb.qrg.noise, 0, t3 * 4u, l3 * 4u);
+      ung[b][j] = AD::ld32(Bb.qng.noise, 0, t3 * 4u, l3 * 4u);
     }
   }
 
@@ -253,7 +254,7 @@
   for (int j = 0; j < J; ++j) {
     if (NQ % kBThreads && wu * 64 + j * kBThreads >= NQ) break;
     const int pix = (tid + j * kBThreads) / C4;
-    const uint32_t off = (uint32_t)(row0 * W * C + pix * C + cq);
+    const uint32_t t3 = (uint32_t)row0 * kRowB + j * 4 * kBThreads;
     const float4 t = *reinterpret_cast<const float4*>(sh.tile + pix * (C + 4) + cq);
     pf2 g[2] = {pk(t.x, t.y), pk(t.z, t.w)};
     if (has_add) {
@@ -276,7 +277,8 @@
         g[h] = pk(yv.x > 0.f ? g[h].x : 0.f, yv.y > 0.f ? g[h].y : 0.f);
       }
     }
-    if (CF & kAGmask) st_out4(A.gmask_out, (uint32_t)(img + off), make_float4(g[0].x, g[0].y, g[1].x, g[1].y));
+    if (CF & kAGmask)
+      AD::st32(A.gmask_out, img, t3 * 4u, l3 * 4u, make_float4(g[0].x, g[0].y, g[1].x, g[1].y));
 #pragma unroll
     for (int b = 0; b < NB; ++b) {
       const lbt_bwd_branch& Bb = b == 0 ? A.b1 : A.b2;
@@ -307,7 +309,7 @@
           acc3[b][3][k] += Gc[k] * qn[k];
         }
       }
-      st_out(Bb.gout + img + off, pack4_i8(Gc));
+      AD::st8(Bb.gout, img, t3, l3, pack4_i8(Gc));
     }
   }
 
@@ -370,7 +372,7 @@
   const int C = d.Cin;
   if (!desc_ok(d) || d.KH != 3 || d.KW != 3 || d.SH != 1 || d.SW != 1 || d.PT != 1 || d.PB != 1 || d.PL != 1 ||
       d.PR != 1 || d.Ho != d.H || d.Wo != d.W || d.Cout != C || (C != 16 && C != 32 && C != 64) ||
-      d.H % tile_rows(C / 16) || d.W * C != 512 || (int64_t)d.N * d.H * 512 >= ((int64_t)1 << 29))
+      d.H % tile_rows(C / 16) || d.W * C != 512 || !fused_extent_ok(d.N, d.H))
     return LBT_EINVAL;
   const int CS = C / 16;
   const int64_t inner = (int64_t)d.H * d.W * C;
@@ -842,7 +844,7 @@
       d1.PL != 0 || ds.KH != 1 || ds.KW != 1 || ds.SH != 2 || ds.SW != 2 || ds.PT != 0 || ds.PL != 0 ||
       (C != 16 && C != 32) || Cq != 2 * C || d1.W * C != 512 || d1.H % 2 || d1.W % 2 || d1.Ho * 2 != d1.H ||
       d1.Wo * 2 != d1.W || d1.H % tile_rows(C / 16) || ds.N != d1.N || ds.H != d1.H || ds.W != d1.W || ds.Cin != C ||
-      ds.Cout != Cq || ds.Ho != d1.Ho || ds.Wo != d1.Wo || (int64_t)d1.N * d1.H * 512 >= ((int64_t)1 << 29))
+      ds.Cout != Cq || ds.Ho != d1.Ho || ds.Wo != d1.Wo || !fused_extent_ok(d1.N, d1.H))
     return LBT_EINVAL;
   const int CS = C / 16;
   const int64_t inq = (int64_t)d1.Ho * d1.Wo * Cq;
diff --git a/lbt_amd/csrc/conv_fused_fwd.h b/lbt_amd/csrc/conv_fused_fwd.h
--- a/lbt_amd/csrc/conv_fused_fwd.h
+++ b/lbt_amd/csrc/conv_fused_fwd.h
@@ -29,14 +29,16 @@
   int cnt[INF ? 1 : kBNW * 2 * 4];
 };
 
-__host__ __device__ constexpr int fwd_waves(int CS, int NB, bool W4, int TH, bool INF) {
-  return (CS == 4 && TH >= 4) ? 2 : (CS == 2 && NB == 2 && W4 && TH == 2 && !INF) ? 6 : 4;
+__host__ __device__ constexpr int fwd_waves(int CS, int NB, bool W4, int TH, bool INF, int F) {
+  return (CS == 4 && TH >= 4) ? 2 : (CS == 2 && NB == 2 && W4 && TH == 2 && !INF) ? 6
+         : (CS == 1 && NB == 1 && TH == 2 && !INF && (F & kFY) && !(F & kFRes)) ? 8 : 4;
 }
 template <int CS, int NB, int F, bool W4, int TH = tile_rows(CS), bool INF = false>
-__global__ __launch_bounds__(kBThreads, fwd_waves(CS, NB, W4, TH, INF)) void conv_fwd_fused_kernel(ConvFwdArgs p) {
+__global__ __launch_bounds__(kBThreads, fwd_waves(CS, NB, W4, TH, INF, F)) void conv_fwd_fused_kernel(ConvFwdArgs p) {
   using T = FusedTile<CS, TH>;
   constexpr int C = T::C, C4 = T::C4, NT = T::NT, W = T::W, Wp = T::Wp, kMaxKS = T::kMaxKS;
   constexpr int kBIt = T::kBIt, NQ = T::NQ, J = T::J, NPR = T::NPR;
+  using AD = Addr<!(CS == 4 && NB == 2)>;
   using WI = WImg<C, 4 * kMaxKS, W4>;
   __shared__ __attribute__((aligned(16))) FwdShared<C, TH, WI::kBytes, INF> sh;
   LBT_TS(0);
@@ -44,11 +46,13 @@
   const int H = p.H;
   const uint32_t bid = blockIdx.x;
   const int tpi = H / TH;
-  const int n = (int)(bid / (uint32_t)tpi), row0 = (int)(bid - (uint32_t)n * tpi) * TH;
+  const int n = uni((int)(bid / (uint32_t)tpi)), row0 = uni((int)(bid - (uint32_t)n * tpi) * TH);
   const int tid = threadIdx.x, lane = tid & 63, wave = tid >> 6;
   const int r = lane & 15, kg = lane >> 4;
   const int cq = (tid % C4) * 4;
-  const int64_t img = (int64_t)n * H * W * C;
+  const int64_t img = (int64_t)n * H * kRowB;
+  const int wu = wave_id();
+  const uint32_t l1 = lane_off1();
   constexpr bool RES = (F & kFRes) != 0, YST = (F & kFY) != 0;
 
   static_assert(LBT_NSHARD == 32 && kBThreads == 512 && (NB * C) % 16 == 0 && NB * C / 16 <= kBNW,
@@ -77,16 +81,16 @@
   float4 rv[kBIt], nrv[NB][kBIt], nov[kBIt];
 #pragma unroll
   for (int it = 0; it < kBIt; ++it) {
-    const int g = tid + it * kBThreads;
-    const uint32_t off = g < ngrp ? (uint32_t)((ylo * W + g / C4) * C + cq) : 0u;
+    const int gw = it * kBThreads + wu * 64;
+    const uint32_t rowb = gw < ngrp ? (uint32_t)(ylo + gw / 128) * kRowB : 0u;
 #pragma unroll
     for (int b = 0; b < NB; ++b) {
       const lbt_chain_branch& Bb = b == 0 ? a.b1 : a.b2;
-      qv[b][it] = ld_i8x4(Bb.nrm.q, img + off);
-      nrv[b][it] = ld_f32x4(Bb.qr.noise, off);
-    }
-    if constexpr (RES) rv[it] = ld_f32x4(a.res, img + off);
-    nov[it] = ld_f32x4(a.qo1.noise, off);
+      qv[b][it] = AD::ld8(Bb.nrm.q, img, rowb, l1);
+      nrv[b][it] = AD::ld32(Bb.qr.noise, 0, rowb * 4u, l1 * 4u);
+    }
+    if constexpr (RES) rv[it] = AD::ld32(a.res, img, rowb * 4u, l1 * 4u);
+    nov[it] = AD::ld32(a.qo1.noise, 0, rowb * 4u, l1 * 4u);
   }
   v4i wimg[WI::kIt];
   WI::load(p.wf, wimg);
@@ -167,20 +171,15 @@
       bet2[b][h] = pk(bet[b][2 * h], bet[b][2 * h + 1]);
     }
 
-  int wu = wave;
-  if constexpr (!INF) wu = __builtin_amdgcn_readfirstlane(wave);
   int ovr[2] = {0, 0}, ovx = 0;
 #pragma unroll
   for (int it = 0; it < kBIt; ++it) {
-    if (it * kBThreads + wu * 64 >= ngrp) break;
-    const int g = tid + it * kBThreads;
-    const int ry = g / (W * C4), x = g / C4 - ry * W;
-    const int y = ylo + ry, hy = y - row0 + 1;
-    const int pix = hy * Wp + x + 1;
+    const int gw = it * kBThreads + wu * 64;
+    if (gw >= ngrp) break;
+    const int y = ylo + gw / 128, hy = y - row0 + 1;
     const bool own = hy >= 1 && hy <= TH;
-    const int hyw = ylo + (it * kBThreads + wu * 64) / (W * C4) - row0 + 1;
-    const int nanw = hyw >= 1 && hyw <= TH ? 0 : kOvNan;
-    const uint32_t e = (uint32_t)((y * W + x) * C + cq);
+    const int nanw = own ? 0 : kOvNan;
+    const uint32_t e = (uint32_t)y * kRowB;
     pf2 v[2];
     float T1[2], T2[2];
     if constexpr (!INF) {
@@ -210,7 +209,7 @@
         const pf2 tt = m1 + bet2[b][h];
         v[h] = b ? v[h] + tt : tt;
       }
-      if (own && (!INF || Bb.rout)) st_out(Bb.rout + img + e, pack4f(fl[0], fl[1]));
+      if (own && (!INF || Bb.rout)) AD::st8(Bb.rout, img, e, l1, pack4f(fl[0], fl[1]));
     }
     if constexpr (RES) {
       v[0] = v[0] + pk(rv[it].x, rv[it].y);
@@ -218,7 +217,7 @@
     }
 #pragma unroll
     for (int h = 0; h < 2; ++h) v[h] = pk(v[h].x > 0.f ? v[h].x : 0.f, v[h].y > 0.f ? v[h].y : 0.f);
-    if (YST && own) st_out4(a.y, (uint32_t)(img + e), make_float4(v[0].x, v[0].y, v[1].x, v[1].y));
+    if (YST && own) AD::st32(a.y, img, e * 4u, l1 * 4u, make_float4(v[0].x, v[0].y, v[1].x, v[1].y));
     const pf2 uo[2] = {pk(nov[it].x, nov[it].y), pk(nov[it].z, nov[it].w)};
     const float X1 = ov_thr(nanw, so1.L), X2 = ov_thr(nanw, so1.Lh);
     int co[4];
@@ -231,18 +230,19 @@
       co[2 * h + 1] = floor_i(fminf(w.y, so1.Lm1));
     }
     const int cw = pack4_i8(co) ^ (int)0x80808080;
-    *reinterpret_cast<int*>(sh.x + pix * C + cq) = cw;
-    if (own && (!INF || a.o1)) st_out((int8_t*)a.o1 + img + e, cw);
+    *reinterpret_cast<int*>(sh.x + (hy * Wp + 1) * C + l1) = cw;
+    if (own && (!INF || a.o1)) AD::st8((int8_t*)a.o1, img, e, l1, cw);
   }
   halo_pad_fill<C, TH>(sh.x, row0, H, (int)0x80808080);
   WI::store(sh.w, wimg);
   __syncthreads();
   LBT_TS(2);
   float4 u3[J];
+  const uint32_t l3 = (NQ % kBThreads && tid >= NQ) ? (uint32_t)cq : (uint32_t)tid * 4u;
 #pragma unroll
   for (int j = 0; j < J; ++j) {
-    const int q3 = tid + j * kBThreads;
-    u3[j] = ld_f32x4(p.qout.noise, (uint32_t)(row0 * W * C + ((q3 < NQ ? q3 : 0) / C4) * C + cq));
+    const uint32_t t3 = (uint32_t)row0 * kRowB + j * 4 * kBThreads;
+    u3[j] = AD::ld32(p.qout.noise, 0, t3 * 4u, l3 * 4u);
   }
 
 #pragma unroll
@@ -274,7 +274,7 @@
   int s1[4] = {0, 0, 0, 0}, s2[4] = {0, 0, 0, 0};
 #pragma unroll
   for (int j = 0; j < J; ++j) {
-    if (NQ % kBThreads && (INF ? tid : wu * 64) + j * kBThreads >= NQ) break;
+    if (NQ % kBThreads && wu * 64 + j * kBThreads >= NQ) break;
     const int pix3 = (tid + j * kBThreads) / C4;
     const float4 t = *reinterpret_cast<const float4*>(sh.tile + pix3 * (C + 4) + cq);
     const pf2 tv[2] = {pk(t.x, t.y), pk(t.z, t.w)};
@@ -294,7 +294,7 @@
         s2[k] += c[k] * c[k];
       }
     }
-    st_out(p.yq + img + (uint32_t)(row0 * W * C + pix3 * C + cq), pack4_i8(c));
+    AD::st8(p.yq, img, (uint32_t)row0 * kRowB + j * 4 * kBThreads, l3, pack4_i8(c));
   }
   if constexpr (!INF) {
     {
diff --git a/lbt_amd/csrc/conv_fused_fwd.hip b/lbt_amd/csrc/conv_fused_fwd.hip
--- a/lbt_amd/csrc/conv_fused_fwd.hip
+++ b/lbt_amd/csrc/conv_fused_fwd.hip
@@ -31,7 +31,7 @@
   const int C = d.Cin;
   if (!desc_ok(d) || d.KH != 3 || d.KW != 3 || d.SH != 1 || d.SW != 1 || d.PT != 1 || d.PB != 1 || d.PL != 1 ||
       d.PR != 1 || d.Ho != d.H || d.Wo != d.W || d.Cout != C || (C != 16 && C != 32 && C != 64) ||
-      d.H % tile_rows(C / 16) || d.W * C != 512 || (int64_t)d.N * d.H * 512 >= ((int64_t)1 << 29))
+      d.H % tile_rows(C / 16) || d.W * C != 512 || !fused_extent_ok(d.N, d.H))
     return LBT_EINVAL;
   const int CS = C / 16;
   const lbt_chain_fwd& a = q->c;
@@ -99,7 +99,7 @@
       d1.PL != 0 || ds.KH != 1 || ds.KW != 1 || ds.SH != 2 || ds.SW != 2 || ds.PT != 0 || ds.PL != 0 ||
       (C != 16 && C != 32) || Cq != 2 * C || d1.W * C != 512 || d1.H % 2 || d1.W % 2 || d1.Ho * 2 != d1.H ||
       d1.Wo * 2 != d1.W || d1.Ho % kTH2 || ds.N != d1.N || ds.H != d1.H || ds.W != d1.W || ds.Cin != C ||
-      ds.Cout != Cq || ds.Ho != d1.Ho || ds.Wo != d1.Wo || (int64_t)d1.N * d1.H * 512 >= ((int64_t)1 << 29))
+      ds.Cout != Cq || ds.Ho != d1.Ho || ds.Wo != d1.Wo || !fused_extent_ok(d1.N, d1.H))
     return LBT_EINVAL;
   const int CS = C / 16;
   const lbt_chain_fwd& a = q->c;
diff --git a/lbt_amd/csrc/conv_fused_infer.hip b/lbt_amd/csrc/conv_fused_infer.hip
--- a/lbt_amd/csrc/conv_fused_infer.hip
+++ b/lbt_amd/csrc/conv_fused_infer.hip
@@ -18,7 +18,7 @@
   const int C = d.Cin;
   if (!desc_ok(d) || d.KH != 3 || d.KW != 3 || d.SH != 1 || d.SW != 1 || d.PT != 1 || d.PB != 1 || d.PL != 1 ||
       d.PR != 1 || d.Ho != d.H || d.Wo != d.W || d.Cout != C || (C != 16 && C != 32 && C != 64) ||
-      d.H % tile_rows(C / 16) || d.W * C != 512 || (int64_t)d.N * d.H * 512 >= ((int64_t)1 << 29))
+      d.H % tile_rows(C / 16) || d.W * C != 512 || !fused_extent_ok(d.N, d.H))
     return LBT_EINVAL;
   const int CS = C / 16;
   const lbt_chain_fwd& a = q->c;
@@ -74,7 +74,7 @@
       d1.PL != 0 || ds.KH != 1 || ds.KW != 1 || ds.SH != 2 || ds.SW != 2 || ds.PT != 0 || ds.PL != 0 ||
       (C != 16 && C != 32) || Cq != 2 * C || d1.W * C != 512 || d1.H % 2 || d1.W % 2 || d1.Ho * 2 != d1.H ||
       d1.Wo * 2 != d1.W || d1.Ho % kTH2 || ds.N != d1.N || ds.H != d1.H || ds.W != d1.W || ds.Cin != C ||
-      ds.Cout != Cq || ds.Ho != d1.Ho || ds.Wo != d1.Wo || (int64_t)d1.N * d1.H * 512 >= ((int64_t)1 << 29))
+      ds.Cout != Cq || ds.Ho != d1.Ho || ds.Wo != d1.Wo || !fused_extent_ok(d1.N, d1.H))
     return LBT_EINVAL;
   const int CS = C / 16;
   const lbt_chain_fwd& a = q->c;
diff --git a/lbt_amd/csrc/dfxp_device.h b/lbt_amd/csrc/dfxp_device.h
--- a/lbt_amd/csrc/dfxp_device.h
+++ b/lbt_amd/csrc/dfxp_device.h
@@ -364,6 +364,23 @@
 
 LBT_DEV int ld_i8x4(const int8_t* p, int64_t i) { return *reinterpret_cast<const int*>(p + i); }
 LBT_DEV float4 ld_f32x4(const float* p, int64_t i) { return *reinterpret_cast<const float4*>(p + i); }
+LBT_DEV __amdgpu_buffer_rsrc_t ubuf(const void* base) {
+  return __builtin_amdgcn_make_buffer_rsrc(const_cast<void*>(base), 0, 0x7fffffff, 0x00020000);
+}
+LBT_DEV int ld_i8x4_u(const int8_t* base, uint32_t sbyte, uint32_t vbyte) {
+  return (int)__builtin_amdgcn_raw_buffer_load_b32(ubuf(base), (int)vbyte, (int)sbyte, 0);
+}
+LBT_DEV float4 ld_f32x4_u(const float* base, uint32_t sbyte, uint32_t vbyte) {
+  const auto v = __builtin_amdgcn_raw_buffer_load_b128(ubuf(base), (int)vbyte, (int)sbyte, 0);
+  return make_float4(__uint_as_float(v[0]), __uint_as_float(v[1]), __uint_as_float(v[2]), __uint_as_float(v[3]));
+}
+LBT_DEV void st_out_u(int8_t* base, uint32_t sbyte, uint32_t vbyte, int v) {
+#ifdef LBT_PLAIN_OUT
+  __builtin_amdgcn_raw_buffer_store_b32((unsigned)v, ubuf(base), (int)vbyte, (int)sbyte, 0);
+#else
+  __builtin_amdgcn_raw_buffer_store_b32((unsigned)v, ubuf(base), (int)vbyte, (int)sbyte, 16 );
+#endif
+}
 LBT_DEV void unpack4_i8(int w, int v[4]) {
   v[0] = (int8_t)(w & 0xff); v[1] = (int8_t)((w >> 8) & 0xff);
   v[2] = (int8_t)((w >> 16) & 0xff); v[3] = (int8_t)(w >> 24);
```

New measurement: 335,600 samples/s, median of 4. 2.9% higher.
